# wuyakuma/HIPRT-Path-Tracer

Hardware: AMD Instinct MI355X
Metric: Mray/s + Msample/s, Bistro 1920×1080, 1/2/4/8 MI355X; RMSE vs ref @256spp (higher is better)
Workload: dtype f32

## Files before the change

hiprt-path-tracer_amd/csrc/mpt_api.cpp:

```cpp
#include <dlfcn.h>
#include <hip/hip_runtime.h>

#include <algorithm>
#include <cfloat>
#include <cmath>
#include <cstdio>
#include <cstdlib>
#include <cstring>
#include <deque>
#include <mutex>
#include <string>
#include <vector>

#include "bvh8.h"
#include "denoise.h"
#include "display.h"
#include "mpt.h"
#include "mpt_internal.h"
#include "refit.h"

using namespace mpt;

namespace {

// ... 49 lines not shown

constexpr int FRAME_RING = 256;
constexpr int PIX_PARTS_MAX = 4;
constexpr int RESTIR_MAX_BATCH = 128;
constexpr int EV_POOL = 2 * 2 * ((10 * 65 + 3 + 8) > 50 * RESTIR_MAX_BATCH ? (10 * 65 + 3 + 8) : 50 * RESTIR_MAX_BATCH);
constexpr int SPILL_WORDS = 2 * TRAV_SPILL_DEPTH;
constexpr int MAX_STACK = TRAV_LDS_STACK + TRAV_SPILL_DEPTH;

}

struct MptContext {
    int device = 0;
    hipStream_t stream = nullptr;
    bool own_stream = false;
    int overlap = -1;
    hipStream_t stream2 = nullptr;
    hipStream_t streamx[2] = {nullptr, nullptr};
    hipEvent_t ev_joinx[2] = {nullptr, nullptr};
    hipEvent_t ev_fork = nullptr, ev_first = nullptr, ev_acc = nullptr, ev_join = nullptr;
    int restir_overlap = 1;
    bool restir_overlap_ok = false;
    int restir_half = 0;
    hipEvent_t ev_chain = nullptr, ev_half[2] = {nullptr, nullptr}, ev_wave_join = nullptr;
    bool ev_half_used[2] = {false, false};
    bool wave_pending = false;
    int graphs = 0;
    int pix_parts = 3;
    int restir_side = 1;
    hipEvent_t ev_side[2] = {nullptr, nullptr};
    int trace_ahead = 1;
    int ovl_ahead = 1;
    hipEvent_t ev_ahead[2] = {nullptr, nullptr};
    hipEvent_t ev_ahead2[2] = {nullptr, nullptr};
    uint32_t ahead_launches = 0;
    uint32_t pipelined_batches = 0;
    hipGraphExec_t graph_exec = nullptr;
    std::vector<uint8_t> graph_key;
    uint32_t graph_launches = 0;
    uint32_t graph_captures = 0, graph_replays = 0;
    uint32_t overlapped_batches = 0;
    int num_cus = 256;
    int grid = 1024;
    bool has_scene = false;
    BVH8 bvh;
    DBuf<Node8> nodes;
    DBuf<TriRec> tris;
    DBuf<float4> tri_attr;
    DBuf<float> srgb;
    BVH8 bvh_light;
    DBuf<Node8> nodes_light;
    DBuf<TriRec> tris_light;
    std::vector<int32_t> h_light_prims;
    std::vector<int32_t> h_idx;
    std::vector<float> h_pos;
    float box_pad = 0.0f;
    DBuf<float> nbox, nbox_light, tbox;
    double area0 = 0.0, area0_light = 0.0;
    bool mirrors_stale = false;
    bool topology_stale = false;
    std::vector<uint8_t> h_vert_used;
    int refit_host_loop = 0;
    int light_bvh = 1;
    bool light_bvh_ok = false;
    int light_bvh_max_stack = 1 << 30;
    DBuf<int32_t> idx, mat_idx, mat_prio, emissive, tex_dims;
    DBuf<float> pos, nrm, uv;
    DBuf<uint8_t> has_n, tex;
    DBuf<uint64_t> tex_off;
    DBuf<MptMaterial> mats;
    DBuf<MptMaterial> mats_res;
    DBuf<int32_t> mat_tex;
    DBuf<float4> em_tab;
    bool any_tex = false;
    bool any_glass = false;
    double tex_tri_frac = 0.0;
    int mat_private = -1;
    int shade_classes = 1;
    int restir_staged = 1;
    int restir_mono_reuse = 0;
    int restir_batch = 1;
    int adaptive_batch = 1;
    int restir_max_batch = RESTIR_MAX_BATCH;
    int shade_glass = 1;
    int shade_split = 0;
    int shade_texmetal = 1;
    std::vector<MptMaterial> h_mats;
    std::vector<int32_t> h_mat_idx;
    std::vector<uint8_t> h_tex_alpha;
    int n_tex = 0;
    DBuf<float> lut_conductor, lut_glossy, lut_glass, lut_glass_inv, lut_thin, lut_sheen;
    DBuf<float4> env;
    DBuf<int2> alias;
    DBuf<float4> env_rich;
    DBuf<float> env_cdf;
    float env_cdf_sum = 0.0f;
    int env_w = 0, env_h = 0;
    float env_sum = 0.0f;
    int res_x = 0, res_y = 0, band_h = 1, band_i = 0, band_c = 1, n_slots = 0;
    int batch_cap = 0;
    int batch = 1;
    DBuf<float4> ray_o, ray_d, hit, thr, col, alb, nrmv, nq_o, nq_d, nhit, s_gn;
    DBuf<uint8_t> hit_inside, hit_cls, occ, qmask;
    DBuf<uint32_t> rng, spill, spill2, spillx[2];
    DBuf<uint2> seeds;
    DBuf<uint4> vsA, vsB;
    DBuf<int32_t> q0, q1, qh, qm, qf, nq_light, counters, nq_tgt, fetch_raw;
    DBuf<float4> nthr, na, nb, ndir, nris, ne1, ne2;
    DBuf<float4> nthr2, na2, nb2, ndir2, nris2, ne12, ne22, nq_o2, nq_d2, ce, ce2;
    DBuf<int32_t> nq_tgt2, qh2, qf2;
    int pipeline = 1;
    size_t pipe_n = 0;
    hipEvent_t ev_nee[4] = {nullptr, nullptr, nullptr, nullptr};
    int pix_pipe = 1;
    DBuf<float> fb_color, fb_albedo, fb_normal;
    DBuf<int32_t> as_count, as_conv;
    DBuf<float> as_sqlum;
    DBuf<uint8_t> active;
    DBuf<uint32_t> status;
    DBuf<float4> gb_pos, gb_sn, gb_gn, gb_view, pgb_pos, pgb_sn, pgb_gn, pgb_view;
    DBuf<int4> gb_meta, pgb_meta;
    DBuf<uint4> gb_vsA, gb_vsB, pgb_vsA, pgb_vsB;
    DBuf<MptMaterial> gb_mat, pgb_mat;
    DBuf<float4> gb_cs, pgb_cs;
    DBuf<float4> rs_init, rs_sp1, rs_sp2, rs_plights;
    DBuf<float4> rs_keep;
    DBuf<int32_t> rs_conv;
    DBuf<float4> rq_o, rq_d, rq_rec;
    DBuf<uint32_t> rq_key;
    DBuf<uint8_t> rq_occ;
    DBuf<int32_t> rq_list, rq_items;
    DBuf<int4> rq_meta;
    int restir_chunk = -1;
    int ci_chunk = 1;
    DBuf<float4> ci_pos, ci_sn, ci_gn, ci_view, ci_cs, ci_rs, ci_pl;
    DBuf<int4> ci_meta;
    DBuf<uint4> ci_vsA, ci_vsB;
    DBuf<MptMaterial> ci_mat;
    DevPaths ci_dp{};
    int restir_out_sp2 = 0;
    MptHaloExchangeFn halo_fn = nullptr;
    void* halo_user = nullptr;
    int halo_prev = 0;
    int32_t* h_reproj = nullptr;
    DBuf<MptMaterial> mat_slot;
    DBuf<float4> xq_o, xq_d, xq_hit, xrec;
    DBuf<uint8_t> xq_occ, xq_flag;
    DBuf<int32_t> xl_any, xl_cl, xl_light;
    int x_per = 0, x_iter = 0;
    DBuf<uint64_t> stats;
    DBuf<uint64_t> ray_counts;
    MptFrame* h_frames = nullptr;
    MptFrame* d_frames = nullptr;
    int frame_slot = 0;
    bool timing = false;
    bool instrumented = false;
    hipEvent_t ev[2][EV_POOL];
    int ev_mode[2][EV_POOL / 2];
    hipEvent_t ev_frame[2][2];
    int ev_used[2] = {0, 0};
    bool ev_pending[2] = {false, false};
    uint32_t frames_submitted = 0;
    uint32_t trace_launches = 0;
    uint32_t frames = 0;
    double stage_ms[KT_COUNT] = {};
    uint32_t stage_launches[KT_COUNT] = {};
    double frame_ms = 0.0;
// ... 619 lines not shown
    return MPT_OK;
}

int mpt_device_info(int device, char* name, int32_t name_cap, char* arch, int32_t arch_cap, int32_t* out_cus) {
    hipDeviceProp_t p;
    HIPCHK(hipGetDeviceProperties(&p, device));
    if (name && name_cap > 0) { std::strncpy(name, p.name, (size_t)name_cap - 1); name[name_cap - 1] = 0; }
    if (arch && arch_cap > 0) { std::strncpy(arch, p.gcnArchName, (size_t)arch_cap - 1); arch[arch_cap - 1] = 0; }
    if (out_cus) *out_cus = p.multiProcessorCount;
    return MPT_OK;
}

static_assert(sizeof(MptMaterial) == 332, "RendererMaterial mirror");
static_assert(sizeof(MptRenderSettings) == 304, "HIPRTRenderSettings mirror");
static_assert(sizeof(MptWorldSettings) == 200, "WorldSettings mirror");
static_assert(sizeof(MptCamera) == 196, "HIPRTCamera mirror");

int mpt_partition_rows(int32_t res_y, int32_t bh, int32_t bi, int32_t bc) {
    if (bh <= 0 || bc <= 0) return 0;
    return rows_of(res_y, bh, bi, bc);
}

static int create_context(MptContext* c, int device, void* hip_stream) {
    c->device = device;
    HIPCHK(hipSetDevice(device));
    hipDeviceProp_t prop;
    HIPCHK(hipGetDeviceProperties(&prop, device));
    c->num_cus = prop.multiProcessorCount;
    c->grid = c->num_cus * MPT_TRACE_BLOCKS_PER_CU;
    if (hip_stream) c->stream = (hipStream_t)hip_stream;
    else { HIPCHK(hipStreamCreateWithFlags(&c->stream, hipStreamNonBlocking)); c->own_stream = true; }
    HIPCHK(hipHostMalloc((void**)&c->h_frames, sizeof(MptFrame) * (FRAME_RING + 1)));
    HIPCHK(hipMalloc((void**)&c->d_frames, sizeof(MptFrame) * (FRAME_RING + 1)));
    HIPCHK(c->counters.alloc(PIX_PARTS_MAX * CTR_COUNT));
    HIPCHK(hipMemsetAsync(c->counters.p, 0, PIX_PARTS_MAX * CTR_COUNT * sizeof(int32_t), c->stream));
    HIPCHK(c->fetch_raw.alloc(4));
    HIPCHK(c->stats.alloc(N_STATS));
    HIPCHK(hipMemsetAsync(c->stats.p, 0, N_STATS * sizeof(uint64_t), c->stream));
    HIPCHK(c->ray_counts.alloc(N_RAY_COUNTS));
    HIPCHK(c->status.alloc(4));
    HIPCHK(hipMemsetAsync(c->status.p, 0, 4 * sizeof(uint32_t), c->stream));
    HIPCHK(hipMemsetAsync(c->ray_counts.p, 0, N_RAY_COUNTS * sizeof(uint64_t), c->stream));
    HIPCHK(c->spill.alloc((size_t)c->num_cus * TRACE_SPILL_BLOCKS_PER_CU * TRAV_BLOCK * SPILL_WORDS));
    HIPCHK(c->srgb.alloc(256));
    HIPCHK(launch_srgb_table(c->srgb.p, c->stream));
    return MPT_OK;
}

static int ensure_events(MptContext* c) {
    for (int p = 0; p < 2; p++) {
        for (int i = 0; i < EV_POOL; i++)
            if (!c->ev[p][i]) HIPCHK(hipEventCreate(&c->ev[p][i]));
        for (int k = 0; k < 2; k++)
            if (!c->ev_frame[p][k]) HIPCHK(hipEventCreate(&c->ev_frame[p][k]));
    }
    return MPT_OK;
}

int mpt_create(int device, void* hip_stream, MptContext** out) {
    if (!out) return fail(MPT_ERR_INVALID_ARGUMENT, "out_ctx is NULL");
    int ndev = 0;
    if (hipGetDeviceCount(&ndev) != hipSuccess || ndev <= 0) return fail(MPT_ERR_HIP, "no HIP device available");
    if (device < 0 || device >= ndev) return fail(MPT_ERR_INVALID_ARGUMENT, "device index out of range");
    MptContext* c = new MptContext();
    if (const char* e = std::getenv("MPT_SHADE_CLASSES")) c->shade_classes = std::atoi(e);
    if (const char* e = std::getenv("MPT_RESTIR_STAGED")) c->restir_staged = std::atoi(e);
    if (const char* e = std::getenv("MPT_RESTIR_MONO_REUSE")) c->restir_mono_reuse = std::atoi(e);
    if (const char* e = std::getenv("MPT_RESTIR_BATCH")) c->restir_batch = std::atoi(e);
    if (const char* e = std::getenv("MPT_ADAPTIVE_BATCH")) c->adaptive_batch = std::atoi(e);
    if (const char* e = std::getenv("MPT_MAT_PRIVATE")) c->mat_private = std::atoi(e);
    if (const char* e = std::getenv("MPT_RESTIR_OVERLAP")) c->restir_overlap = std::atoi(e);
    if (const char* e = std::getenv("MPT_GRAPHS")) c->graphs = std::atoi(e);
    if (const char* e = std::getenv("MPT_PIX_PARTS")) c->pix_parts = std::atoi(e);
    if (const char* e = std::getenv("MPT_RESTIR_SIDE")) c->restir_side = std::atoi(e);
    if (const char* e = std::getenv("MPT_TRACE_AHEAD")) c->trace_ahead = std::atoi(e);
    if (const char* e = std::getenv("MPT_PIPELINE")) c->pipeline = std::atoi(e);
    if (const char* e = std::getenv("MPT_PIX_PIPE")) c->pix_pipe = std::atoi(e);
    if (const char* e = std::getenv("MPT_OVERLAP_AHEAD")) c->ovl_ahead = std::atoi(e);
    if (const char* e = std::getenv("MPT_RESTIR_MAX_BATCH"))
        c->restir_max_batch = std::max(1, std::min(RESTIR_MAX_BATCH, std::atoi(e)));
    if (const char* e = std::getenv("MPT_RESTIR_CHUNK")) c->restir_chunk = std::atoi(e);
    if (const char* e = std::getenv("MPT_SHADE_GLASS")) c->shade_glass = std::atoi(e);
    if (const char* e = std::getenv("MPT_SHADE_SPLIT")) c->shade_split = std::atoi(e);
    if (const char* e = std::getenv("MPT_SHADE_TEXMETAL")) c->shade_texmetal = std::atoi(e);
    if (const char* e = std::getenv("MPT_LIGHT_BVH")) c->light_bvh = std::atoi(e);
    if (const char* e = std::getenv("MPT_OVERLAP")) c->overlap = std::atoi(e);
    if (const char* e = std::getenv("MPT_LIGHT_BVH_MAX_STACK")) c->light_bvh_max_stack = std::atoi(e);
    if (const char* e = std::getenv("MPT_REFIT_HOST")) c->refit_host_loop = std::atoi(e);
    int r = create_context(c, device, hip_stream);
    if (r != MPT_OK) {
        const std::string msg = g_err;
        mpt_destroy(c);
        g_err = msg;
        return r;
    }
    *out = c;
    return MPT_OK;
}

namespace {
void rccl_comm_destroy(void* comm);
}

int mpt_destroy(MptContext* c) {
    if (!c) return MPT_OK;
    (void)hipSetDevice(c->device);
    if (c->stream) (void)hipStreamSynchronize(c->stream);
    if (c->comm) rccl_comm_destroy(c->comm);
    for (int p = 0; p < 2; p++) {
        for (int i = 0; i < EV_POOL; i++)
            if (c->ev[p][i]) (void)hipEventDestroy(c->ev[p][i]);
        for (int k = 0; k < 2; k++)
            if (c->ev_frame[p][k]) (void)hipEventDestroy(c->ev_frame[p][k]);
    }
    if (c->graph_exec) (void)hipGraphExecDestroy(c->graph_exec);
    if (c->h_frames) (void)hipHostFree(c->h_frames);
    if (c->h_reproj) (void)hipHostFree(c->h_reproj);
    if (c->d_frames) (void)hipFree(c->d_frames);
    if (c->own_stream && c->stream) (void)hipStreamDestroy(c->stream);
    if (c->stream2) (void)hipStreamDestroy(c->stream2);
    for (int k = 0; k < 2; k++) {
        if (c->streamx[k]) (void)hipStreamDestroy(c->streamx[k]);
        if (c->ev_joinx[k]) (void)hipEventDestroy(c->ev_joinx[k]);
        if (c->ev_side[k]) (void)hipEventDestroy(c->ev_side[k]);
        if (c->ev_ahead[k]) (void)hipEventDestroy(c->ev_ahead[k]);
        if (c->ev_ahead2[k]) (void)hipEventDestroy(c->ev_ahead2[k]);
    }
    for (hipEvent_t e : c->ev_nee)
        if (e) (void)hipEventDestroy(e);
    for (hipEvent_t e : {c->ev_fork, c->ev_first, c->ev_acc, c->ev_join, c->ev_chain, c->ev_half[0], c->ev_half[1],
                         c->ev_wave_join})
        if (e) (void)hipEventDestroy(e);
    delete c;
    (void)hipGetLastError();
    return MPT_OK;
}

int mpt_upload_scene(MptContext* c, const MptScene* s) {
    if (!c || !s) return fail(MPT_ERR_INVALID_ARGUMENT, "NULL argument");
    if (s->num_triangles <= 0 || s->num_vertices <= 0 || !s->triangle_indices || !s->vertices || !s->material_indices ||
        !s->materials || s->num_materials <= 0)
        return fail(MPT_ERR_INVALID_ARGUMENT, "scene has no geometry or materials");
    for (int64_t i = 0; i < 3 * (int64_t)s->num_triangles; i++)
        if (s->triangle_indices[i] < 0 || s->triangle_indices[i] >= s->num_vertices)
            return fail(MPT_ERR_INVALID_ARGUMENT, "triangle index out of range");
    for (int64_t i = 0; i < s->num_triangles; i++)
        if (s->material_indices[i] < 0 || s->material_indices[i] >= s->num_materials)
            return fail(MPT_ERR_INVALID_ARGUMENT, "material index out of range");
    for (int i = 0; i < s->num_emissive_triangles; i++)
        if (s->emissive_triangle_indices[i] < 0 || s->emissive_triangle_indices[i] >= s->num_triangles)
            return fail(MPT_ERR_INVALID_ARGUMENT, "emissive triangle index out of range");
    HIPCHK(hipSetDevice(c->device));
    const int stack_cap = build_scene_bvh8(s->vertices, s->triangle_indices, s->num_triangles, c->bvh, MAX_STACK);
    c->box_pad = scene_box_pad(s->vertices, s->num_triangles, s->triangle_indices);
    c->area0 = node_box_area_sum(c->bvh.node_box.data(), c->bvh.nodes.size());
    c->mirrors_stale = false;
    c->topology_stale = false;
    c->h_vert_used.assign((size_t)s->num_vertices, 0);
    for (size_t k = 0; k < 3 * (size_t)s->num_triangles; k++) c->h_vert_used[s->triangle_indices[k]] = 1;
    c->h_idx.assign(s->triangle_indices, s->triangle_indices + 3 * (size_t)s->num_triangles);
    c->h_pos.assign(s->vertices, s->vertices + 3 * (size_t)s->num_vertices);
    c->h_light_prims.clear();
    c->nodes_light.release();
    c->tris_light.release();
    if (2 * c->bvh.depth + 2 > stack_cap) return fail(MPT_ERR_UNSUPPORTED, "BVH8 deeper than the traversal stack");
    hipStream_t st = c->stream;
// ... 437 lines not shown
        return fail(MPT_ERR_INVALID_ARGUMENT, "ReSTIR DI across a partition needs mpt_set_halo_exchange");
    if (f->options.direct_light_sampling == MPT_LSS_RESTIR_DI) {
        r = ensure_restir(c, f);
        if (r != MPT_OK) return r;
    }
    if (f->options.direct_light_sampling == MPT_LSS_RESTIR_DI && c->emissive.n == 0 &&
        (f->options.restir_di_later_bounces_sampling_strategy == MPT_RESTIR_DI_LATER_BOUNCES_UNIFORM_ONE_LIGHT ||
         f->options.restir_di_later_bounces_sampling_strategy == MPT_RESTIR_DI_LATER_BOUNCES_MIS_LIGHT_BSDF))
        return fail(MPT_ERR_UNSUPPORTED, "ReSTIR DI later bounces: uniform / MIS light sampling without emissive "
                                         "triangles picks from an empty list in the reference (Lights.h:22-220)");
    if ((int64_t)std::max(c->n_slots, 1) * batch > MPT_MAX_WAVEFRONT_PATHS)
        return fail(MPT_ERR_OUT_OF_MEMORY, "wavefront above MPT_MAX_WAVEFRONT_PATHS paths");
    const MptRenderSettings& frs = f->render_settings;
    const bool adaptive = (frs.stop_pixel_noise_threshold > 0.0f || frs.enable_adaptive_sampling) && frs.accumulate;
    const bool want_overlap = f->options.direct_light_sampling == MPT_LSS_RESTIR_DI && batch > 1 && c->restir_overlap &&
                              !(adaptive && c->as_reset_pending) &&
                              ext_layout(*f, nullptr) == 0 && (int64_t)std::max(c->n_slots, 1) * 2 * batch <= MPT_MAX_WAVEFRONT_PATHS;
    c->restir_overlap_ok = false;
    if (want_overlap) {
        const int cap = 2 * batch;
        r = ensure_batch(c, cap, c->any_tex || f->bsdf_flags.white_furnace_mode);
        if (r == MPT_OK) c->restir_overlap_ok = c->batch_cap / 2 >= batch;
        else { (void)hipGetLastError(); g_err.clear(); }
    }
    if (!c->restir_overlap_ok) {
        r = ensure_batch(c, batch, c->any_tex || f->bsdf_flags.white_furnace_mode);
        if (r != MPT_OK) return r;
    }
    const bool keep = f->options.direct_light_sampling == MPT_LSS_RESTIR_DI &&
                      f->world_settings.ambient_light_type == MPT_AMBIENT_ENVMAP;
    if (!keep && c->rs_keep.p) {
        HIPCHK(drain(c));
        c->rs_keep.release();
    }
    const size_t keep_n = 3 * (size_t)std::max(c->n_slots, 1) * (size_t)(c->restir_overlap_ok ? c->batch_cap : batch);
    if (keep && batch > 1 && c->rs_keep.n < keep_n) {
        HIPCHK(drain(c));
        c->rs_keep.release();
        if (c->rs_keep.alloc(keep_n) != hipSuccess) {
            (void)hipGetLastError();
            return fail(MPT_ERR_OUT_OF_MEMORY, "ReSTIR DI batch reservoirs");
        }
    }
    int iter = 0;
    const int per = ext_layout(*f, &iter);
    return ensure_ext(c, batch, per, iter);
}

static int ensure_overlap(MptContext* c) {
    if (c->stream2) return MPT_OK;
    if (c->spill2.n != c->spill.n) HIPCHK(c->spill2.alloc(c->spill.n));
    for (hipEvent_t* e : {&c->ev_fork, &c->ev_first, &c->ev_acc, &c->ev_join, &c->ev_chain, &c->ev_half[0], &c->ev_half[1],
                          &c->ev_wave_join})
        if (!*e) HIPCHK(hipEventCreateWithFlags(e, hipEventDisableTiming));
    HIPCHK(hipStreamCreateWithFlags(&c->stream2, hipStreamNonBlocking));
    return MPT_OK;
}

static int join_waves(MptContext* c);

static int ensure_pix_parts(MptContext* c, int parts) {
    int r = ensure_overlap(c);
    if (r != MPT_OK) return r;
    for (int k = 0; k + 2 < parts; k++) {
        if (c->spillx[k].n != c->spill.n) HIPCHK(c->spillx[k].alloc(c->spill.n));
        if (!c->ev_joinx[k]) HIPCHK(hipEventCreateWithFlags(&c->ev_joinx[k], hipEventDisableTiming));
        if (!c->streamx[k]) HIPCHK(hipStreamCreateWithFlags(&c->streamx[k], hipStreamNonBlocking));
    }
    return MPT_OK;
}

static hipError_t launch_frame_graph(MptContext* c, const DevPaths& P, const MptFrame* f, int slot, LaunchCfg& cfg) {
    const DevScene S = dev_scene(c);
    MptFrame k = *f;
    k.random_seed = 0;
    k.camera_random_seed = 0;
    std::memset(k.restir_di_seeds, 0, sizeof(k.restir_di_seeds));
    std::memset(&k.current_camera, 0, sizeof(MptCamera));
    std::memset(&k.prev_camera, 0, sizeof(MptCamera));
    k.render_settings.sample_number = 0;
    k.render_settings.denoiser_AOV_accumulation_counter = 0;
    k.render_settings.need_to_reset = false;
    k.render_settings.do_update_status_buffers = false;
    const int flags[9] = {cfg.grid_persistent, cfg.stats, cfg.shade_classes, cfg.light_bvh, cfg.light_static,
                          cfg.restir_staged, cfg.shade_glass, cfg.shade_split, cfg.mat_private};
    std::vector<uint8_t> key(sizeof(k) + sizeof(S) + sizeof(P) + sizeof(flags));
    uint8_t* q = key.data();
    std::memcpy(q, &k, sizeof(k)); q += sizeof(k);
    std::memcpy(q, &S, sizeof(S)); q += sizeof(S);
    std::memcpy(q, &P, sizeof(P)); q += sizeof(P);
    std::memcpy(q, flags, sizeof(flags));
    MptFrame* d_fixed = c->d_frames + FRAME_RING;
    hipError_t e = hipMemcpyAsync(d_fixed, c->h_frames + slot, sizeof(MptFrame), hipMemcpyHostToDevice, c->stream);
    if (e != hipSuccess) return e;
    if (!c->graph_exec || key != c->graph_key) {
        if (c->graph_exec) { (void)hipGraphExecDestroy(c->graph_exec); c->graph_exec = nullptr; }
        hipGraph_t g = nullptr;
        e = hipStreamBeginCapture(c->stream, hipStreamCaptureModeThreadLocal);
        if (e != hipSuccess) return e;
        LaunchCfg gc = cfg;
        gc.launches = 0;
        const hipError_t le = launch_frame(S, P, d_fixed, *f, gc, c->stream);
        e = hipStreamEndCapture(c->stream, &g);
        if (le != hipSuccess || e != hipSuccess) {
            if (g) (void)hipGraphDestroy(g);
            (void)hipGetLastError();
            c->graphs = 0;
            return launch_frame(S, P, c->d_frames + slot, *f, cfg, c->stream);
        }
        e = hipGraphInstantiate(&c->graph_exec, g, nullptr, nullptr, 0);
        (void)hipGraphDestroy(g);
        if (e != hipSuccess) {
            c->graph_exec = nullptr;
            (void)hipGetLastError();
            c->graphs = 0;
            return launch_frame(S, P, c->d_frames + slot, *f, cfg, c->stream);
        }
        c->graph_key = std::move(key);
        c->graph_launches = gc.launches;
        c->graph_captures++;
    }
    cfg.launches += c->graph_launches;
    c->graph_replays++;
    return hipGraphLaunch(c->graph_exec, c->stream);
}

static bool is_reset(const MptFrame& f) { return f.render_settings.sample_number == 0 || f.render_settings.need_to_reset; }
static bool has_adaptive(const MptFrame& f) {
    const MptRenderSettings& rs = f.render_settings;
    return (rs.stop_pixel_noise_threshold > 0.0f || rs.enable_adaptive_sampling) && rs.accumulate;
}
static int next_as_bound(int b, const MptFrame& f) {
    if (!has_adaptive(f)) return b;
    if (is_reset(f)) b = 0;
    return b < (1 << 30) ? b + 1 : b;
}
static bool note_conv_set(bool set, int bound, const MptFrame& f) {
    if (!has_adaptive(f)) return set;
    const MptRenderSettings& rs = f.render_settings;
    if (is_reset(f)) { set = false; bound = 0; }
    if (rs.enable_adaptive_sampling) return set || bound > rs.adaptive_sampling_min_samples;
    return set || (rs.enable_pixel_stop_noise_threshold && rs.sample_number > 1);
}
static int set_ahead(MptContext* c, LaunchCfg& cfg, const MptFrame& f, int which = 0) {
    if (!c->trace_ahead || f.render_settings.nb_bounces <= 0) return MPT_OK;
    int rr = ensure_pix_parts(c, 4);
    if (rr != MPT_OK) return rr;
    hipEvent_t* evs = which ? c->ev_ahead2 : c->ev_ahead;
    for (int k = 0; k < 2; k++)
        if (!evs[k]) HIPCHK(hipEventCreateWithFlags(&evs[k], hipEventDisableTiming));
    cfg.ahead_stream = which ? c->streamx[0] : c->streamx[1];
    cfg.ahead_spill = which ? c->spillx[0].p : c->spillx[1].p;
    cfg.ev_ahead_fork = evs[0];
    cfg.ev_ahead_join = evs[1];
    return MPT_OK;
}

static bool pipe_applies(const MptContext* c, const MptFrame& f) {
    return c->pipeline && f.options.direct_light_sampling != MPT_LSS_RESTIR_DI && c->x_per == 0 && !c->shade_split &&
           f.render_settings.nb_bounces > 0;
}
static int set_pipe(MptContext* c, LaunchCfg& cfg, const MptFrame& f, DevPaths& P, DevPaths& alt, int part = -1,
                    size_t off = 0) {
    if (!pipe_applies(c, f)) return MPT_OK;
    const size_t N = (size_t)std::max(c->n_slots, 1) * (size_t)c->batch_cap;
    if (c->pipe_n != N) {
        HIPCHK(drain(c));
        Allocs A;
// ... 18 lines not shown
    alt = P;
    alt.nthr = c->nthr2.p; alt.na = c->na2.p; alt.nb = c->nb2.p; alt.ndir = c->ndir2.p; alt.nris = c->nris2.p;
    alt.ne1 = c->ne12.p; alt.ne2 = c->ne22.p; alt.nq_o = c->nq_o2.p; alt.nq_d = c->nq_d2.p; alt.nq_tgt = c->nq_tgt2.p;
    alt.qh = c->qh2.p; alt.qf = c->qf2.p; alt.ce = c->ce2.p;
    if (off) {
        alt.nthr += off; alt.na += off; alt.nb += off; alt.ndir += off; alt.nris += off; alt.ne1 += off; alt.ne2 += off;
        alt.nq_o += off; alt.nq_d += off; alt.nq_tgt += 4 * off; alt.qh += off; alt.qf += off; alt.ce += off;
    }
    alt.counters = part < 0 ? P.counters + CTR_COUNT : P.counters + 2 * CTR_COUNT;
    cfg.pipe_alt = &alt;
    cfg.nee_stream = c->streamx[k];
    cfg.nee_spill = c->spillx[k].p;
    cfg.ev_nee_fork = c->ev_nee[2 * k];
    cfg.ev_nee_join = c->ev_nee[2 * k + 1];
    return MPT_OK;
}

static int launch_batch(MptContext* c, const MptFrame* f, int batch) {
    const bool restir_part = f->options.direct_light_sampling == MPT_LSS_RESTIR_DI && f->band_count > 1;
    if (!(f->options.direct_light_sampling == MPT_LSS_RESTIR_DI && batch > 1 && c->restir_overlap_ok)) {
        int jr = join_waves(c);
        if (jr != MPT_OK) return jr;
    }
    const int parts_set = c->pix_pipe && pipe_applies(c, *f) ? std::min(c->pix_parts, 2) : c->pix_parts;
    const int parts = std::min(std::max(parts_set, 1), std::min(PIX_PARTS_MAX, f->res_y));
    const bool pix_ovl = parts > 1 && batch == 1 && f->band_count == 1 && c->n_slots >= (1 << 16) &&
                         f->options.direct_light_sampling != MPT_LSS_RESTIR_DI && c->x_per == 0 &&
                         !(c->graphs && !c->timing);
    const int nfr = batch + (pix_ovl ? parts - 1 : 0);
    if (c->frame_slot + nfr > FRAME_RING) c->frame_slot = 0;
    int slot = c->frame_slot;
    c->frame_slot = (c->frame_slot + nfr) % FRAME_RING;
    if (slot == 0) {
        HIPCHK(hipStreamSynchronize(c->stream));
        if (c->stream2) HIPCHK(hipStreamSynchronize(c->stream2));
    }
    for (int k = 0; k < batch; k++) c->h_frames[slot + k] = f[k];
    const int hp = (f->res_y + parts - 1) / parts;
    if (pix_ovl) {
        for (int k = 1; k < parts; k++) {
            MptFrame& g = c->h_frames[slot + k];
            g = f[0];
            g.band_height = hp;
            g.band_index = k;
            g.band_count = parts;
        }
    }
    HIPCHK(hipMemcpyAsync(c->d_frames + slot, c->h_frames + slot, nfr * sizeof(MptFrame), hipMemcpyHostToDevice,
                          c->stream));
    int pool = (int)(c->frames_submitted & 1u);
    if (c->timing) {
        int rc = collect_pool(c, pool);
        if (rc != MPT_OK) return rc;
    }
    LaunchCfg cfg{};
    cfg.grid_persistent = c->grid;
    cfg.stats = c->instrumented ? 1 : 0;
    cfg.ev_pool = c->timing ? c->ev[pool] : nullptr;
    cfg.ev_mode = c->ev_mode[pool];
    cfg.ev_cap = EV_POOL;
    cfg.ev_used = 0;
    cfg.restir_out_sp2 = c->restir_out_sp2;
    cfg.shade_classes = c->shade_classes;
    cfg.restir_staged = c->restir_staged;
    cfg.restir_mono_reuse = c->restir_mono_reuse;
    if (c->ci_chunk > 1 && c->ci_pos.p && c->ci_pl.n >= 4 * (size_t)std::max(1, f->render_settings.restir_di_settings.number_of_subsets *
                                                                                     f->render_settings.restir_di_settings.subset_size) * c->ci_chunk) {
        cfg.ci_chunk = c->ci_chunk;
        cfg.ci_planes = &c->ci_dp;
    }
    if (f->options.direct_light_sampling == MPT_LSS_RESTIR_DI && c->restir_staged &&
        (c->restir_side > 1 || (c->restir_side == 1 && c->n_slots <= (1 << 20)))) {
        int rr = ensure_pix_parts(c, 3);
        if (rr != MPT_OK) return rr;
        for (hipEvent_t& ev : c->ev_side)
            if (!ev) HIPCHK(hipEventCreateWithFlags(&ev, hipEventDisableTiming));
        cfg.side_stream = c->streamx[0];
        cfg.side_spill = c->spillx[0].p;
        cfg.ev_side_fork = c->ev_side[0];
        cfg.ev_side_join = c->ev_side[1];
    }
    cfg.shade_glass = c->shade_glass && c->any_glass;
    cfg.shade_split = c->shade_split;
    cfg.mat_private = c->mat_private >= 0 ? (c->mat_private != 0) : (c->tex_tri_frac >= 0.25);
    cfg.light_bvh = c->light_bvh && c->light_bvh_ok;
    cfg.light_static = !c->h_light_prims.empty() && 2 * c->bvh_light.depth + 2 <= TRAV_LDS_STACK;
    if (restir_part) {
        if (!c->h_reproj) HIPCHK(hipHostMalloc((void**)&c->h_reproj, sizeof(int32_t), hipHostMallocDefault));
        cfg.halo_fn = c->halo_fn;
        cfg.halo_user = c->halo_user;
        cfg.own_y0 = f->band_index * f->band_height;
        cfg.own_y1 = std::min(f->res_y, cfg.own_y0 + f->band_height);
        cfg.halo_prev = c->halo_prev;
        cfg.halo_rows = c->halo_prev;
        cfg.h_reproj = c->h_reproj;
    }
    if (c->timing) HIPCHK(hipEventRecord(c->ev_frame[pool][0], c->stream));
    c->batch = batch;
    DevPaths P = dev_paths(c);
    c->batch = 1;
    {
        const MptRenderSettings& rs = f->render_settings;
        P.spec_as = batch > 1 && (rs.stop_pixel_noise_threshold > 0.0f || rs.enable_adaptive_sampling) && rs.accumulate;
        P.spec_skip = P.spec_as && rs.enable_adaptive_sampling && c->as_bound > rs.adaptive_sampling_min_samples;
    }
    if (restir_part) {
        P.rs_lo = std::max(0, cfg.own_y0 - cfg.halo_prev) * f->res_x;
        P.rs_hi = std::min(f->res_y, cfg.own_y1 + cfg.halo_prev) * f->res_x;
    }
    const bool pipe_ok = c->pipeline && !c->shade_split && f->render_settings.nb_bounces > 0;
    const bool pipe_first = pipe_ok && c->mat_idx.n >= PIPELINE_PREFER_TRIS;
    const bool ovl_auto = ((size_t)batch * (size_t)std::max(c->n_slots, 1) <= OVERLAP_AUTO_PATHS && !pipe_first) ||
                          (f->render_settings.nb_bounces >= 8 && !pipe_ok);
    const bool ovl = (c->overlap > 0 || (c->overlap < 0 && ovl_auto)) && batch >= 2 &&
                     f->options.direct_light_sampling != MPT_LSS_RESTIR_DI && c->x_per == 0 && !P.spec_as;
    hipError_t e = hipSuccess;
    if (pix_ovl) {
        int rr = ensure_pix_parts(c, parts);
        if (rr != MPT_OK) return rr;
        HIPCHK(hipEventRecord(c->ev_fork, c->stream));
        LaunchCfg cur = cfg;
        int launches = 0;
        const bool part_pipe = c->pix_pipe && parts == 2 && pipe_applies(c, *f);
        DevPaths alts[2];
        for (int k = 0; k < parts && e == hipSuccess; k++) {
            const size_t r0 = std::min((size_t)f->res_y, (size_t)k * hp), r1 = std::min((size_t)f->res_y, (size_t)(k + 1) * hp);
            const size_t off = r0 * (size_t)f->res_x, n = (r1 - r0) * (size_t)f->res_x;
            if (n == 0) continue;
            DevPaths Pk = P;
            Pk.n = Pk.n_pix = (int)n;
            if (k > 0) {
                offset_slots(Pk, off);
                Pk.fb_color += 3 * off; Pk.fb_albedo += 3 * off; Pk.fb_normal += 3 * off;
                Pk.as_count += off; Pk.as_sqlum += off; Pk.as_conv += off;
                Pk.counters += k * CTR_COUNT;
                Pk.stack_spill = k == 1 ? c->spill2.p : c->spillx[k - 2].p;
            }
            hipStream_t sk = k == 0 ? c->stream : k == 1 ? c->stream2 : c->streamx[k - 2];
            if (k > 0) HIPCHK(hipStreamWaitEvent(sk, c->ev_fork, 0));
            cur.pipe_alt = nullptr;
            cur.nee_stream = nullptr;
            if (part_pipe) {
                int rr2 = set_pipe(c, cur, *f, Pk, alts[k], k, k > 0 ? off : 0);
                if (rr2 != MPT_OK) return rr2;
                if (cur.pipe_alt) c->pipelined_batches++;
            }
            cur.launches = 0;
            e = launch_frame(dev_scene(c), Pk, c->d_frames + slot + k, k == 0 ? f[0] : c->h_frames[slot + k], cur, sk);
            launches += cur.launches;
        }
        for (int k = 1; k < parts; k++) {
            hipStream_t sk = k == 1 ? c->stream2 : c->streamx[k - 2];
            hipEvent_t ej = k == 1 ? c->ev_join : c->ev_joinx[k - 2];
            HIPCHK(hipEventRecord(ej, sk));
            HIPCHK(hipStreamWaitEvent(c->stream, ej, 0));
        }
        c->overlapped_batches++;
        cfg.ev_used = cur.ev_used;
        cfg.launches = launches;
    } else if (ovl) {
        int rr = ensure_overlap(c);
        if (rr != MPT_OK) return rr;
        const int b0 = batch / 2, b1 = batch - b0;
        c->batch = b0;
        DevPaths P0 = dev_paths(c);
        c->batch = b1;
// ... 559 lines not shown
        const int p0 = std::min(res_y, p * bh), p1 = std::min(res_y, p0 + bh);
        int c0, c1, d0, d1, lo, hi;
        const bool theirs = need(p, c0, c1, d0, d1);
        for (int i = 0; i < n_buffers; i++) {
            if (theirs && band_overlap(c0, c1, m0, m1, lo, hi)) ops.push_back({p, 0, i, lo, hi});
            if (theirs && band_overlap(d0, d1, m0, m1, lo, hi)) ops.push_back({p, 0, i, lo, hi});
            if (mine && band_overlap(a0, a1, p0, p1, lo, hi)) ops.push_back({p, 1, i, lo, hi});
            if (mine && band_overlap(b0, b1, p0, p1, lo, hi)) ops.push_back({p, 1, i, lo, hi});
        }
    }
}
int native_halo(void* user, MptHaloExchange* x) {
    MptContext* c = (MptContext*)user;
    hipStream_t st = (hipStream_t)x->stream;
    std::vector<MptHaloOp>& ops = c->halo_plan_ops;
    auto count = [&](int recv) {
        size_t bytes = 0;
        for (const MptHaloOp& o : ops)
            if (o.recv == recv) bytes += (size_t)(o.row_hi - o.row_lo) * (size_t)x->res_x * (size_t)x->bytes_per_pixel[o.buffer];
        return bytes;
    };
    if (c->halo_native == 2) {
        if (x->phase == MPT_HALO_GBUFFER && !x->halo_agreed && hipStreamSynchronize(st) != hipSuccess) return 1;
        halo_ops(x->res_y, c->band_h, std::max(1, c->band_c), c->band_i, x->halo_rows, x->n_buffers, ops);
        const size_t bytes = count(1);
        c->halo_exchanges++;
        c->halo_bytes_recv += bytes;
        c->halo_bytes_sent += count(0);
        if (bytes == 0) return 0;
        if (c->halo_scratch.n < 2 * bytes && c->halo_scratch.alloc(2 * bytes) != hipSuccess) return 1;
        return hipMemcpyAsync(c->halo_scratch.p + bytes, c->halo_scratch.p, bytes, hipMemcpyDeviceToDevice, st) == hipSuccess ? 0 : 1;
    }
    Rccl& r = *rccl_lib();
    if (!c->comm || !r.send || !r.recv || !r.group_start || !r.group_end || !r.all_reduce) return 2;
    const int n = c->comm_size, k = c->comm_rank;
    if (c->band_c != n || c->band_i != k) return 4;
    if (x->phase == MPT_HALO_GBUFFER && !x->halo_agreed) {
        if (c->halo_agree.n < 1 && c->halo_agree.alloc(1) != hipSuccess) return 1;
        int32_t v = x->halo_rows;
        if (hipMemcpyAsync(c->halo_agree.p, &v, sizeof(v), hipMemcpyHostToDevice, st) != hipSuccess) return 1;
        if (r.all_reduce(c->halo_agree.p, c->halo_agree.p, 1, NCCL_INT32, NCCL_MAX, c->comm, st) != 0) return 3;
        if (hipMemcpyAsync(&v, c->halo_agree.p, sizeof(v), hipMemcpyDeviceToHost, st) != hipSuccess ||
            hipStreamSynchronize(st) != hipSuccess) return 1;
        x->halo_rows = v;
        c->halo_agreements++;
    }
    halo_ops(x->res_y, c->band_h, n, k, x->halo_rows, x->n_buffers, ops);
    c->halo_exchanges++;
    c->halo_bytes_recv += count(1);
    c->halo_bytes_sent += count(0);
    if (ops.empty()) return 0;
    int rc = r.group_start();
    for (size_t j = 0; j < ops.size() && rc == 0; j++) {
        const MptHaloOp& o = ops[j];
        uint8_t* buf = (uint8_t*)x->buffers[o.buffer];
        const size_t row = (size_t)x->res_x * (size_t)x->bytes_per_pixel[o.buffer];
        uint8_t* at = buf + (size_t)o.row_lo * row;
        const size_t len = (size_t)(o.row_hi - o.row_lo) * row;
        rc = o.recv ? r.recv(at, len, NCCL_UINT8, o.peer, c->comm, st) : r.send(at, len, NCCL_UINT8, o.peer, c->comm, st);
    }
    const int re = r.group_end();
    return rc != 0 ? 3 : (re != 0 ? 3 : 0);
}
}

int mpt_halo_plan(int32_t res_y, int32_t band_height, int32_t band_count, int32_t band_index, int32_t halo_rows,
                  int32_t n_buffers, MptHaloOp* out, int32_t cap) {
    if (res_y <= 0 || band_height <= 0 || band_count <= 0 || band_index < 0 || band_index >= band_count || halo_rows < 0 ||
        n_buffers < 0 || n_buffers > MPT_HALO_MAX_BUFFERS || cap < 0 || (cap > 0 && !out))
        return fail(MPT_ERR_INVALID_ARGUMENT, "mpt_halo_plan: bad partition, halo or output");
    std::vector<MptHaloOp> ops;
    halo_ops(res_y, band_height, band_count, band_index, halo_rows, n_buffers, ops);
    for (size_t j = 0; j < ops.size() && (int32_t)j < cap; j++) out[j] = ops[j];
    return (int)ops.size();
}

int mpt_set_pipeline(MptContext* c, int32_t mode) {
    if (!c) return fail(MPT_ERR_INVALID_ARGUMENT, "NULL context");
    if (mode < 0 || mode > 1) return fail(MPT_ERR_INVALID_ARGUMENT, "mode must be 0 (in line) or 1 (pipelined)");
    c->pipeline = mode;
    return MPT_OK;
}

int mpt_set_halo_native(MptContext* c, int32_t mode) {
    if (!c) return fail(MPT_ERR_INVALID_ARGUMENT, "NULL context");
    if (mode < 0 || mode > 2) return fail(MPT_ERR_INVALID_ARGUMENT, "mode must be 0 (off), 1 (RCCL) or 2 (rehearsal)");
    if (mode == 1) {
        if (!c->comm) return fail(MPT_ERR_INVALID_ARGUMENT, "no communicator (mpt_comm_init)");
        Rccl& r = *rccl_lib();
        if (!r.send || !r.recv || !r.group_start || !r.group_end || !r.all_reduce)
            return fail(MPT_ERR_UNSUPPORTED, "librccl.so.1 lacks ncclSend / ncclRecv / ncclGroupStart / ncclAllReduce");
    }
    c->halo_native = mode;
    c->halo_fn = mode ? &native_halo : nullptr;
    c->halo_user = mode ? (void*)c : nullptr;
    return MPT_OK;
}

int mpt_clear_status(MptContext* c) {
    if (!c) return fail(MPT_ERR_INVALID_ARGUMENT, "NULL context");
    HIPCHK(hipSetDevice(c->device));
    HIPCHK(hipMemsetAsync(c->status.p, 0, 4 * sizeof(uint32_t), c->stream));
    return MPT_OK;
}

int mpt_query_status(MptContext* c, MptStatus* out) {
    if (!c || !out) return fail(MPT_ERR_INVALID_ARGUMENT, "NULL argument");
    HIPCHK(hipSetDevice(c->device));
    uint32_t v[4];
    HIPCHK(hipMemcpyAsync(v, c->status.p, sizeof(v), hipMemcpyDeviceToHost, c->stream));
    HIPCHK(hipStreamSynchronize(c->stream));
    out->one_ray_active = v[1] != 0;
    out->pixel_converged_count = v[0];
    return MPT_OK;
}

int mpt_get_aux_buffer(MptContext* c, int kind, void* dst, int dst_is_device) {
    if (!c || !dst) return fail(MPT_ERR_INVALID_ARGUMENT, "NULL argument");
    const void* src = kind == MPT_AUX_SAMPLE_COUNT ? (const void*)c->as_count.p
                    : kind == MPT_AUX_CONVERGED_SAMPLE_COUNT ? (const void*)c->as_conv.p
                    : kind == MPT_AUX_SQUARED_LUMINANCE ? (const void*)c->as_sqlum.p : nullptr;
    size_t bytes = (size_t)c->n_slots * 4;
    if (kind >= MPT_AUX_RESTIR_OUTPUT && kind <= MPT_AUX_RESTIR_INITIAL && c->rs_init.p) {
        const int o = c->restir_out_sp2;
        const float4* out = o == 1 ? c->rs_sp2.p : o == 2 ? c->rs_init.p : c->rs_sp1.p;
        src = kind == MPT_AUX_RESTIR_OUTPUT ? (const void*)out
            : kind == MPT_AUX_RESTIR_OTHER ? (const void*)(o == 1 ? c->rs_sp1.p : c->rs_sp2.p) : (const void*)c->rs_init.p;
        bytes = c->rs_init.n * sizeof(float4);
    }
    if (!src) return fail(MPT_ERR_INVALID_ARGUMENT, "bad aux buffer kind or no frame rendered");
    HIPCHK(hipSetDevice(c->device));
    HIPCHK(hipMemcpyAsync(dst, src, bytes, dst_is_device ? hipMemcpyDeviceToDevice : hipMemcpyDeviceToHost, c->stream));
    HIPCHK(hipStreamSynchronize(c->stream));
    return MPT_OK;
}

int mpt_enable_stats(MptContext* c, int enable, int instrumented) {
    if (!c) return fail(MPT_ERR_INVALID_ARGUMENT, "NULL context");
    HIPCHK(hipSetDevice(c->device));
    HIPCHK(hipStreamSynchronize(c->stream));
    if (enable) {
        int r = ensure_events(c);
        if (r != MPT_OK) { c->timing = false; return r; }
    }
    c->timing = enable != 0;
    c->instrumented = instrumented != 0;
    c->ev_pending[0] = c->ev_pending[1] = false;
    c->trace_launches = 0;
    c->frames = 0;
    c->frame_ms = 0.0;
    c->graph_captures = c->graph_replays = 0;
    c->overlapped_batches = 0;
    c->halo_exchanges = c->halo_agreements = c->halo_bytes_sent = c->halo_bytes_recv = 0;
    c->restir_overlapped_batches = 0;
    c->ahead_launches = 0;
    c->pipelined_batches = 0;
    for (int m = 0; m < KT_COUNT; m++) { c->stage_ms[m] = 0.0; c->stage_launches[m] = 0; }
    HIPCHK(hipMemsetAsync(c->stats.p, 0, N_STATS * sizeof(uint64_t), c->stream));
    HIPCHK(hipMemsetAsync(c->ray_counts.p, 0, N_RAY_COUNTS * sizeof(uint64_t), c->stream));
    HIPCHK(hipStreamSynchronize(c->stream));
    return MPT_OK;
}

int mpt_get_stats(MptContext* c, MptStats* out) {
    if (!c || !out) return fail(MPT_ERR_INVALID_ARGUMENT, "NULL argument");
    HIPCHK(hipSetDevice(c->device));
// ... 157 lines not shown
```

hiprt-path-tracer_amd/csrc/mpt_internal.h:

```cpp
#ifndef MPT_INTERNAL_H
#define MPT_INTERNAL_H

#include <hip/hip_runtime.h>
#include <stdint.h>

#include "bvh8.h"
#include "mpt.h"

namespace mpt {

constexpr int TRAV_BLOCK = 256;
#ifndef MPT_LDS_STACK
#define MPT_LDS_STACK 12
#endif
constexpr int TRAV_LDS_STACK = MPT_LDS_STACK;
constexpr int TRAV_SPILL_DEPTH = 64 - TRAV_LDS_STACK;

#ifndef MPT_TRACE_BLOCKS_PER_CU
#define MPT_TRACE_BLOCKS_PER_CU 5
#endif
#ifndef MPT_TRACE_WAVES
#define MPT_TRACE_WAVES 5
#endif
#ifndef MPT_TRACE_WAVES_LIST
// ... 102 lines not shown
    float4* nq_d;
    int64_t nq_stride;
    int32_t* nq_tgt;
    uint8_t* qmask;
    uint8_t* occ;
    float4* nhit;
    float4* s_gn;
    MptMaterial* mat_slot;
    float4* ce;
    float* fb_color;
    float* fb_albedo;
    float* fb_normal;
    uint32_t* stack_spill;
    uint64_t* stats;
    uint64_t* ray_counts;
    int32_t* as_count;
    float* as_sqlum;
    int32_t* as_conv;
    uint8_t* active;
    int32_t spec_as;
    int32_t spec_reset;
    int32_t spec_skip;
    uint32_t* status;
    float4* gb_pos;
    float4* gb_sn;
    float4* gb_gn;
    float4* gb_view;
    int4* gb_meta;
    uint4* gb_vsA;
    uint4* gb_vsB;
    MptMaterial* gb_mat;
    float4* pgb_pos; float4* pgb_sn; float4* pgb_gn; float4* pgb_view; int4* pgb_meta;
    uint4* pgb_vsA; uint4* pgb_vsB; MptMaterial* pgb_mat;
    float4* gb_cs; float4* pgb_cs;
    float4* rs_init;
    float4* rs_sp1;
    float4* rs_sp2;
    float4* rs_out;
    float4* rs_tin;
    float4* rs_keep;
    int64_t rs_keep_n;
    int rs_keep_on;
    int32_t cam_noqueue;
    float4* rs_plights;
    int32_t pix_off;
    int32_t rs_lo, rs_hi;
    int32_t ci_n;
    int32_t ci_pix_off;
    int32_t* rs_conv;
    int32_t x_per;
    int32_t x_iter;
    float4* xq_o;
    float4* xq_d;
    float4* xq_hit;
    uint8_t* xq_occ;
    uint8_t* xq_flag;
    float4* xrec;
    int32_t* xl_any;
    int32_t* xl_cl;
    int32_t* xl_light;
    float4* rq_o;
    float4* rq_d;
    uint32_t* rq_key;
    uint8_t* rq_occ;
    int32_t* rq_list;
    int32_t* rq_items;
    int4* rq_meta;
    float4* rq_rec;
};

constexpr int N_TRACE_MODES = 5;
constexpr int RS_KMAX_HOST = 5, RS_RPP_HOST = 2 * RS_KMAX_HOST + 2, RS_REC_HOST = RS_KMAX_HOST + 2;
constexpr int N_RAY_COUNTS = 6;
enum { KT_CAMERA = 3, KT_SHADE = 4, KT_RESOLVE = 5, KT_ACCUMULATE = 6, KT_COMPACT = 7, KT_RESTIR = 8, KT_SPLIT = 9,
       KT_MISS = 10, KT_SHADE_GENERIC = 11,
       KT_GBUFFER = 12, KT_RS_PRESAMPLE = 13, KT_RS_INITIAL = 14, KT_RS_REUSE = 15, KT_RS_SPATIAL = 16,
       KT_RS_EVAL = 17, KT_COUNT = 18 };
constexpr uint32_t QM_CONT = 16u;
constexpr int32_t MT_TEXTURED = 1, MT_FULL = 2, MT_GLASS = 4;
constexpr int32_t MT_TEXMETAL = 8;
constexpr int STATS_STRIDE = 6;
constexpr int N_STATS = N_TRACE_MODES * STATS_STRIDE;

enum {
    CTR_Q0 = 0, CTR_Q1 = 1,
    CTR_QG = 2,
    CTR_ANY = 3, CTR_CL = 4,
    CTR_FETCH = 5,
    CTR_REPROJ = 6,
    CTR_HIT = 7, CTR_MISS = 8,
    CTR_FULL = 9,
    CTR_DEFER = 10,
    CTR_LIGHT = 11,
    CTR_XANY = 12, CTR_XCL = 13, CTR_XLIGHT = 14,
    CTR_RQ = 15, CTR_RQV = 16,
    CTR_RQE0 = 17, CTR_RQE1 = 18,
    CTR_F_RQA = 19, CTR_F_RQB = 20,
    CTR_RQ_GROUP = 6,
    CTR_GLASS = 21,
    CTR_F_PATH = 22, CTR_F_ANY = 23, CTR_F_CL = 24, CTR_F_OCC = 25, CTR_F_XANY = 26, CTR_F_XCL = 27, CTR_F_XOCC = 28,
    CTR_COUNT = 29
};
constexpr int CTR_BOUNCE_FIRST = CTR_ANY;

struct LaunchCfg {
    int grid_persistent;
    int stats;
    hipEvent_t* ev_pool;
    int* ev_mode;
    int ev_cap;
    int ev_used;
    uint32_t launches;
    int restir_out_sp2;
    MptHaloExchangeFn halo_fn;
    void* halo_user;
    int own_y0, own_y1;
    int halo_prev;
    int halo_rows;
    int32_t* h_reproj;
    int halo_rc;
    int shade_classes;
    int light_bvh;
    int light_static;
    int restir_staged;
    int restir_mono_reuse;
    int shade_glass;
    int mat_private;
    int shade_split;
    hipEvent_t ev_first_trace;
    hipEvent_t ev_acc_done;
    hipEvent_t ev_acc_wait;
    hipStream_t wave_stream;
    uint32_t* wave_spill;
    hipEvent_t ev_chain;
    hipStream_t side_stream;
    uint32_t* side_spill;
    hipEvent_t ev_side_fork, ev_side_join;
    hipStream_t ahead_stream;
    uint32_t* ahead_spill;
    hipEvent_t ev_ahead_fork, ev_ahead_join;
    uint32_t ahead_launches;
    hipStream_t nee_stream;
    uint32_t* nee_spill;
    hipEvent_t ev_nee_fork, ev_nee_join;
    const DevPaths* pipe_alt;
    int ci_chunk;
    const DevPaths* ci_planes;
};

inline void offset_slots(DevPaths& P, size_t off) {
    P.ray_o += off; P.ray_d += off; P.hit += off; P.hit_inside += off; P.hit_cls += off; P.rng += off; P.seeds += off; P.thr += off; P.col += off;
    P.vsA += off; P.vsB += off; P.alb += off; P.nrm += off;
    P.q0 += off; P.q1 += off; P.qh += off; P.qm += off; P.qf += off; P.nq_light += off;
    P.nthr += off; P.na += off; P.nb += off; P.ndir += off; P.nris += off; P.ne1 += off; P.ne2 += off;
    P.nq_o += off; P.nq_d += off; P.occ += off; P.nq_tgt += 4 * off;
    P.nhit += off; P.s_gn += off; P.qmask += off; P.active += off;
    if (P.mat_slot) P.mat_slot += off;
    if (P.ce) P.ce += off;
}

hipError_t launch_frame(const DevScene& S, const DevPaths& P, const MptFrame* d_frame, const MptFrame& h_frame,
                        LaunchCfg& cfg, hipStream_t st);
hipError_t launch_frames_restir(const DevScene& S, const DevPaths& P, const MptFrame* d_frames, const MptFrame* h_frames,
                                int batch, LaunchCfg& cfg, hipStream_t st);
hipError_t launch_resolve_materials(const DevScene& S, MptMaterial* out_res, int32_t* out_tex, int n, float4* em_tab,
                                   hipStream_t st);
hipError_t launch_restir_fill(float4* reservoirs, int n, hipStream_t st);
hipError_t launch_restir_fill_lights(float4* lights, int n, hipStream_t st);
hipError_t launch_bake(int kind, int w, int h, int d, int ipk, int nb_samples, int iteration, float* out, hipStream_t st);
hipError_t launch_tri_attr(const DevScene& S, float4* out, hipStream_t st);
hipError_t launch_srgb_table(float* out, hipStream_t st);
hipError_t launch_env_rich(const DevScene& S, float4* out, hipStream_t st);
hipError_t launch_display(const MptDisplaySettings& S, const float* src, const float* src2, const int32_t* cnt, int W,
                          int rows, uint32_t* dst, hipStream_t st);
size_t denoise_scratch_floats(int64_t pixels);
hipError_t launch_denoise(const MptDenoiseSettings& S, const float* color, const float* albedo, const float* normals,
                          int W, int H, float* scratch, float* dst, hipStream_t st);
hipError_t launch_refit_tris(TriRec* tris, int n, const int32_t* idx, const float* pos, float pad, float* tbox, hipStream_t st);
hipError_t launch_refit_levels(Node8* nodes, float* node_box, const float* tbox, const int32_t* level_begin, int levels,
                               hipStream_t st);
int build_scene_bvh8(const float* vertices, const int32_t* indices, int32_t num_triangles, BVH8& out, int stack_limit);
int copy_bvh_out(const Node8* nodes, size_t n_nodes, const TriRec* tris, size_t n_tris, int levels, void* out_nodes,
                 int64_t nodes_cap, void* out_tris, int64_t tris_cap, int32_t* out_counts);
struct LbvhDevice {
    Node8* nodes = nullptr;
    TriRec* tris = nullptr;
    float* nbox = nullptr;
    int n_nodes = 0, n_tris = 0, depth = 0;
    std::vector<int32_t> level_begin;
};
struct PlocStats {
    int iterations = 0, tail_iterations = 0;
};
hipError_t build_lbvh_device(const int32_t* d_prims, int n, int n_scene_prims, const int32_t* idx, const float* pos, float pad,
                             const TriRec* old_tris, int n_old, float* tbox, LbvhDevice& out, hipStream_t st, int mode = 0,
                             PlocStats* stats = nullptr);
void free_lbvh(LbvhDevice& o);
hipError_t scan_u64(uint64_t* a, int n, uint64_t* partial, hipStream_t st);
struct PlocScratch {
    int32_t* cref[2];
    int32_t* ccnt[2];
    float* cbox[2];
    int32_t* mate;
    uint64_t* words;
    uint64_t* partial;
    int32_t* count;
    int32_t* tail_info;
};
hipError_t ploc_tree_device(int n, const float* pbox, const uint32_t* order, int32_t* left, int32_t* right, int32_t* first,
                            int32_t* last, float* nbox, uint32_t* order_out, const PlocScratch& B, hipStream_t st,
// ... 33 lines not shown
```

hiprt-path-tracer_amd/csrc/mpt_kernels.hip:

```cpp
#include <hip/hip_runtime.h>

#include <cfloat>
#include <cstring>
#include <initializer_list>
#include <type_traits>
#include <utility>

#include "dev_bsdf.h"
#include "mpt_internal.h"

namespace mpt {

constexpr int TB = TRAV_BLOCK;
constexpr int MAX_BOUNDARY_SKIPS = 16;
#ifndef MPT_TRACE_REFILL
#define MPT_TRACE_REFILL 32
#endif
#ifndef MPT_TRACE_BUDGET
#define MPT_TRACE_BUDGET 16
#endif
constexpr int TRACE_REFILL = MPT_TRACE_REFILL;
constexpr int TRACE_BUDGET = MPT_TRACE_BUDGET;
#ifndef MPT_TRACE_CHUNK
#define MPT_TRACE_CHUNK 256
// ... 1134 lines not shown
                    x_rec(P, ew, make_float4(fw_.r, fw_.g, fw_.b, maxr(0.0f, dot(sn, Lw))), make_float4(0.0f, 0.0f, 0.0f, 0.0f));
                    fw |= XQ_REC;
                    if (vis && ism != 1.0f) x_query(P, ew, true, ep2, prim, Lw, dw - 1.0e-4f, fw);
                }
                if (!vis) {
                    const float cw = inner ? w * target / lpdf : 0.0f;
                    wsum += cw;
                    if (r < cw / wsum) { win = c; win_L = Lw; win_d = dw; }
                }
                P.xq_flag[e] = f0;
                P.xq_flag[ew] = fw;
            }
            if (!vis && win >= 0) {
                uint8_t fw = XQ_REC;
                x_query(P, e0 + nl + win, true, ep2, prim, win_L, win_d - 1.0e-4f, fw);
                P.xq_flag[e0 + nl + win] = fw;
            }
            for (int b = 0; b < nbc; b++) {
                uint8_t fb = 0;
                const size_t e = e0 + 2 * nl + b;
                const float pdf = x_bsdf_cand<OVR, FULL>(P, bc, m, vs, pe, e, prim, ip, sn, gn, view, ism, ep, true, 0.0f, rng, fb);
                const float r = rng();
                if (pdf > 0.0f) P.xrec[2 * e + 1].y = r;
                else x_rec(P, e, make_float4(0.0f, 0.0f, 0.0f, 0.0f), make_float4(0.0f, r, 0.0f, 0.0f));
                P.xq_flag[e] = fb | XQ_REC;
            }
        }
    }
}

DEV void store3(float* p, Col c) { p[0] = c.r; p[1] = c.g; p[2] = c.b; }
DEV void store3(float* p, v3 c) { p[0] = c.x; p[1] = c.y; p[2] = c.z; }
DEV Col load3c(const float* p) { return col(p[0], p[1], p[2]); }
DEV v3 load3v(const float* p) { return mk3(p[0], p[1], p[2]); }

#ifdef MPT_SECTION_TIMING
static __device__ unsigned long long g_sect[8];
#define SECT_BEGIN() uint64_t sect_[6] = {0, 0, 0, 0, 0, 0}; uint64_t tprev_ = __builtin_amdgcn_s_memtime()
#define SECT(k) do { uint64_t now_ = __builtin_amdgcn_s_memtime(); sect_[k] += now_ - tprev_; tprev_ = now_; } while (0)
#define SECT_END() do { if (sect_[1]) for (int k_ = 0; k_ < 6; k_++) atomicAdd(&g_sect[k_], (unsigned long long)sect_[k_]); atomicAdd(&g_sect[7], 1ull); } while (0)
#else
#define SECT_BEGIN() do {} while (0)
#define SECT(k) do {} while (0)
#define SECT_END() do {} while (0)
#endif

enum : uint32_t { RF_ENVMAP = 1u, RF_BSDF_REFRACTION = 2u, RF_UNOCCLUDED = 4u };
struct RResv { int M; float wsum; float UCW; int tri; v3 point; float target; uint32_t flags; };
DEV RResv rr_default() {
    RResv r;
    r.M = 0; r.wsum = 0.0f; r.UCW = 0.0f; r.tri = -1; r.point = mk3(0.0f, 0.0f, 0.0f); r.target = 0.0f; r.flags = 0u;
    return r;
}
DEV RResv rr_load(const float4* b, int i) {
    float4 a = b[3 * (size_t)i], c = b[3 * (size_t)i + 1], d = b[3 * (size_t)i + 2];
    RResv r;
    r.M = __float_as_int(a.x); r.wsum = a.y; r.UCW = a.z; r.tri = __float_as_int(a.w);
    r.point = mk3(c.x, c.y, c.z); r.target = c.w; r.flags = __float_as_uint(d.x);
    return r;
}
DEV void rr_store(float4* b, int i, const RResv& r) {
    b[3 * (size_t)i] = make_float4(__int_as_float(r.M), r.wsum, r.UCW, __int_as_float(r.tri));
    b[3 * (size_t)i + 1] = make_float4(r.point.x, r.point.y, r.point.z, r.target);
    b[3 * (size_t)i + 2] = make_float4(__uint_as_float(r.flags), 0.0f, 0.0f, 0.0f);
}

DEV Col miss_radiance(const DevScene& S, const MptFrame& F, int bounce, v3 d, Col thr) {
    const MptRenderSettings& rs = F.render_settings;
    const MptWorldSettings& ws = F.world_settings;
    Col sky = col(0.0f);
    if (ws.ambient_light_type == MPT_AMBIENT_UNIFORM || F.bsdf_flags.white_furnace_mode) sky = C3(ws.uniform_light_color);
    else if (ws.ambient_light_type == MPT_AMBIENT_ENVMAP) {
        bool sampled = F.options.envmap_sampling != MPT_ESS_NO_SAMPLING;
        if (!sampled || bounce == 0) {
            sky = eval_env_no_pdf(S, F, d);
            bool unscale = sampled ? !ws.envmap_scale_background_intensity : (!ws.envmap_scale_background_intensity && bounce == 0);
            if (unscale) sky /= ws.envmap_intensity;
        }
    }
    sky = clamp_contrib(sky, rs.envmap_contribution_clamp, true);
    return clamp_contrib(sky * thr, rs.indirect_contribution_clamp, bounce > 0);
}

enum ShadeOp {
    OP_DONE = 0, OP_RIS_LIGHT, OP_RIS_BSDF, OP_RIS_WIN, OP_MIS_LIGHT, OP_MIS_BSDF, OP_UNI_LIGHT, OP_BSDF_LIGHT,
    OP_ENV_LIGHT, OP_ENV_BSDF, OP_CONT, OP_RESTIR
};
enum { SG_LIGHT = 1, SG_ENV = 2, SG_CONT = 4, SG_ALL = 7 };
DEV constexpr int op_group(int op) {
    return op == OP_DONE ? 0 : (op == OP_ENV_LIGHT || op == OP_ENV_BSDF) ? SG_ENV : op == OP_CONT ? SG_CONT : SG_LIGHT;
}
template <int ST>
DEV int stage_op(int op, bool do_env, bool do_cont) {
    if (!(ST & SG_LIGHT) && op_group(op) == SG_LIGHT) op = do_env ? OP_ENV_LIGHT : (do_cont ? OP_CONT : OP_DONE);
    if (!(ST & SG_ENV) && op_group(op) == SG_ENV) op = do_cont ? OP_CONT : OP_DONE;
    if (!(ST & SG_CONT) && op == OP_CONT) op = OP_DONE;
    return op;
}

struct ShadeArgs {
    DevScene S;
    DevPaths P;
    const MptFrame* F;
    int bounce;
    int last_bounce;
    int32_t* q_cur;
    const int32_t* count_cur;
    int32_t* q_defer;
    int32_t* count_defer;
    int force_defer;
    int rev;
    int mat_private;
};

#ifndef MPT_PLAIN_SAMPLE_PE
#define MPT_PLAIN_SAMPLE_PE 1
#endif
#ifndef MPT_SHADE_WAVES
#define MPT_SHADE_WAVES 2
#endif
#ifndef MPT_SHADE_PEP
#define MPT_SHADE_PEP 0
#endif
#ifndef MPT_SHADE_WAVES_PLAIN
#define MPT_SHADE_WAVES_PLAIN MPT_SHADE_WAVES
#endif
#define OPIS(X) ((ST & op_group(X)) && op == (X))
#ifndef MPT_SHADE_WAVES_LATE
#define MPT_SHADE_WAVES_LATE 3
#endif
#ifndef MPT_SHADE_PE_LDS_LATE
#define MPT_SHADE_PE_LDS_LATE 0
#endif
template <int OVR, bool PLAIN, bool EXT = false, bool GLASS = false, int ST = SG_ALL, bool MATP = false>
__global__ __launch_bounds__(TB) __attribute__((amdgpu_waves_per_eu(
    !(ST & SG_LIGHT) ? MPT_SHADE_WAVES_LATE : (PLAIN ? MPT_SHADE_WAVES_PLAIN : MPT_SHADE_WAVES)))) void k_shade(ShadeArgs A) {
    constexpr int CLS = PLAIN ? BC_PLAIN : (GLASS ? BC_GLASS : BC_FULL);
    constexpr bool PE_PLAIN = MPT_SHADE_PEP && PLAIN && OVR == MPT_BSDF_NONE && !EXT;
    constexpr bool FIRST = (ST & SG_LIGHT) != 0;
    constexpr bool LAST = (ST & SG_CONT) != 0;
    static_assert(!EXT || ST == SG_ALL, "extended light sampling shades in one stage");
    const DevScene& S = A.S;
    const DevPaths& P = A.P;
    const MptFrame& F = *A.F;
    const MptRenderSettings& rs = F.render_settings;
    const int bounce = A.bounce;
    const int count = *A.count_cur;
    if ((int)(blockIdx.x * TB) >= count) return;
    int i = blockIdx.x * TB + threadIdx.x;
    bool valid = i < count;
    int slot = valid ? (A.rev ? A.q_cur[-1 - i] : A.q_cur[i]) : 0;
    if (!FIRST && slot < 0) { valid = false; slot = 0; }

    BCtx bc;
    bc.mats = S.mats;
    bc.luts = DevLuts{S.lut_conductor, S.lut_glossy, S.lut_glass, S.lut_glass_inv, S.lut_thin_glass, S.lut_sheen};
    bc.clearcoat_comp = F.bsdf_flags.clearcoat_compensation_approximation;
    bc.masking = F.bsdf_flags.ggx_masking_shadowing;

    bool cont = false;
    SECT_BEGIN();
    if (valid) {
        float4 ro = ld_s(&P.ray_o[slot]), rdv = ld_s(&P.ray_d[slot]), hv = ld_s(&P.hit[slot]);
        v3 o = mk3(ro.x, ro.y, ro.z), d = mk3(rdv.x, rdv.y, rdv.z);
        int prim = (int)__float_as_uint(hv.w);
        bool found = prim >= 0;
        VState vs = vs_load_s(P.vsA, P.vsB, slot);
        Rng rng = make_rng(ld_s(&P.rng[slot]));
        const float4 thv = ld_s(&P.thr[slot]);
        Col thr = col(thv.x, thv.y, thv.z);
        const Col thr_vertex = thr;
        Col rcol = col(0.0f);
        if (!P.ce) {
            const float4 cv = ld_s(&P.col[slot]);
            rcol = col(cv.x, cv.y, cv.z);
        }
        v3 ip = mk3(0, 0, 0), gn = mk3(0, 0, 0), sn = mk3(0, 0, 0);
        const Mat* mp = S.mats_res;
        bool mat_in_slot = false;
        constexpr bool MAT_PRIV = MATP && ST == SG_ALL;
        Mat mat_priv;
        if (!FIRST) {
            const float4 ra = ld_s(&P.nhit[slot]), rb = ld_s(&P.s_gn[slot]);
            sn = mk3(ra.x, ra.y, ra.z);
            gn = mk3(rb.x, rb.y, rb.z);
            const int mref = __float_as_int(ra.w);
            mp = mref < 0 ? &P.mat_slot[slot] : &S.mats_res[mref];
            ip = o + hv.x * d;
            if (bounce == 0) d = normalize(d);
        } else if (found) {
            float t = hv.x;
            v2 uv = mk2(hv.y, hv.z);
            ip = o + t * d;
            const HitAttr ha = hit_attributes(S, prim, uv);
            const v2 tc = ha.tc;
            gn = ha.gn;
            sn = ha.sn;
            const int mi = ha.mi;
            if (F.bsdf_flags.white_furnace_mode || (S.mat_tex[mi] & MT_TEXTURED)) {
                if (MAT_PRIV) {
                    mat_priv = intersection_material(S, mi, tc, F.bsdf_flags.white_furnace_mode);
                    mp = &mat_priv;
                } else {
                    P.mat_slot[slot] = intersection_material(S, mi, tc, F.bsdf_flags.white_furnace_mode);
                    mp = &P.mat_slot[slot];
                }
                mat_in_slot = true;
            } else {
                mp = &S.mats_res[mi];
            }
            const Mat& m = *mp;
            bool was_inside = P.hit_inside[slot] != 0;
            if ((!was_inside || m.specular_transmission == 0.0f) && !m.thin_walled) {
                gn *= dot(gn, -d) < 0.0f ? -1.0f : 1.0f;
                sn *= dot(sn, gn) < 0.0f ? -1.0f : 1.0f;
                float NoV = dot(sn, -d);
                sn += (2.0f * clampr(0.0f, 1.0f, -NoV)) * -d;
            }
            if (m.dispersion_scale > 0.0f && m.specular_transmission > 0.0f && vs.wl == 0.0f)
                vs.wl = -(rng() * (float)(830 - 360) + (float)360);
        }
        const Mat& m = *mp;
        if (FIRST && bounce == 0) {
            if (found && is_emissive(m) && dot(-d, gn) < 0) { gn = -gn; sn = -sn; }
            gn = normalize(gn);
            sn = normalize(sn);
            d = normalize(d);
            rng = make_rng(P.seeds[slot].y);
        }
        if (PLAIN && FIRST) {
            const v3 sn_f = (is_emissive(m) && dot(-d, gn) < 0) ? -sn : sn;
            if (!(dot(-d, sn_f) > 0 || m.thin_walled) || m.metallic != 0.0f || A.force_defer || (PE_PLAIN && !plain_vertex_ok(m))) {
                A.q_defer[atomicAdd(A.count_defer, 1)] = slot;
                atomicAdd(&P.counters[CTR_DEFER], 1);
                A.q_cur[i] = -1;
                return;
            }
        }
        uint32_t fl = 0;
        uint32_t qm = 0;
        if (found) {
            if (FIRST && bounce == 0) {
                float4 a = P.alb[slot], n4 = P.nrm[slot];
                P.alb[slot] = make_float4(a.x + m.base_color.r, a.y + m.base_color.g, a.z + m.base_color.b, 0.0f);
                P.nrm[slot] = make_float4(n4.x + sn.x, n4.y + sn.y, n4.z + sn.z, 0.0f);
            }
            if (FIRST && is_emissive(m) && dot(-d, gn) < 0) { gn = -gn; sn = -sn; }
            v3 view = -d;
            if (FIRST) fl |= NF_SHADED;
            const int lss = F.options.direct_light_sampling;
            const MptWorldSettings& ws = F.world_settings;
            const bool restir = lss == MPT_LSS_RESTIR_DI;
            bool do_light = (S.n_emissive != 0 || (restir && ws.ambient_light_type == MPT_AMBIENT_ENVMAP)) &&
                            !(F.bsdf_flags.white_furnace_mode && F.bsdf_flags.white_furnace_mode_turn_off_emissives);
            if (do_light && is_emissive(m)) {
                do_light = false;
                if (FIRST && m.emissive_texture_used && bounce > 0) {
                    fl |= NF_IMM;
                    const Col e = emission_of(m);
                    st_s(&P.na[slot], make_float4(e.r, e.g, e.b, 0.0f));
                }
            }
            do_light = do_light && lss != MPT_LSS_NO_DIRECT_LIGHT_SAMPLING;
            const int lssb = bounce_lss(F, bounce);
            if (restir && bounce > 0 && S.n_emissive == 0 && lssb == MPT_LSS_RIS_BSDF_AND_LIGHT) do_light = false;
            if (FIRST && do_light) fl |= NF_L;
            const bool do_env = ws.ambient_light_type == MPT_AMBIENT_ENVMAP && !F.bsdf_flags.white_furnace_mode &&
                                !is_emissive(m) && ws.envmap_intensity > 0.0f && F.options.envmap_sampling != MPT_ESS_NO_SAMPLING &&
                                !(restir && bounce == 0);
            const bool env_use = lss != MPT_LSS_NO_DIRECT_LIGHT_SAMPLING;
            const bool do_cont = bounce < A.last_bounce;
            const float ism = dot(view, gn) < 0 ? -1.0f : 1.0f;
            const v3 ep = ip + sn * 1.0e-4f * ism;
            const int nl = rs.ris_number_of_light_candidates, nbc = rs.ris_number_of_bsdf_candidates;
            int op = OP_DONE;
            if (do_light) {
                if (restir && bounce == 0) op = OP_RESTIR;
                else if (lssb == MPT_LSS_RIS_BSDF_AND_LIGHT) op = nl > 0 ? OP_RIS_LIGHT : (nbc > 0 ? OP_RIS_BSDF : OP_RIS_WIN);
                else if (lssb == MPT_LSS_MIS_LIGHT_BSDF) op = OP_MIS_LIGHT;
                else if (lssb == MPT_LSS_UNIFORM_ONE_LIGHT) op = OP_UNI_LIGHT;
                else if (lssb == MPT_LSS_BSDF) op = OP_BSDF_LIGHT;
            }
            if (op == OP_DONE) op = do_env ? OP_ENV_LIGHT : (do_cont ? OP_CONT : OP_DONE);
            op = stage_op<ST>(op, do_env, do_cont);
            float wsum = 0.0f, targetW = 0.0f;
            v3 pointW = mk3(0, 0, 0);
            int triW = -1, ris_c = 0;
            bool hasW = false;
            float r_add = 0.0f;
            constexpr bool PE_LDS = (ST & SG_LIGHT) || MPT_SHADE_PE_LDS_LATE;
            using PE = typename std::conditional<PE_PLAIN, PEvalP, PEval>::type;
            __shared__ PE pe_lds[PE_LDS ? TB : 1];
            PE pe_reg;
            PE& pe = PE_LDS ? pe_lds[threadIdx.x] : pe_reg;
            EmPrefetch pf;
            pf.valid = false;
            if (MPT_EM_PREFETCH && (ST & SG_LIGHT) && (op == OP_RIS_LIGHT || op == OP_MIS_LIGHT || op == OP_UNI_LIGHT)) pf.issue(S, rng);
            SECT(0);
            bsdf_eval_pre<OVR, CLS>(bc, m, vs, view, sn, pe);
            SECT(5);
            if constexpr (EXT) {
                if (do_light && !(restir && bounce == 0)) {
                    ext_light<OVR, CLS>(S, P, F, bc, m, vs, pe, slot, prim, ip, sn, gn, view, ism, ep, lssb, rng);
                    fl |= NF_EXT;
                    op = do_env ? OP_ENV_LIGHT : (do_cont ? OP_CONT : OP_DONE);
                }
            }
            Col fW = col(0.0f);
            float pdfW = 0.0f;
            while (op != OP_DONE) {
                VState tv = vs;
                RResv rres;
                v3 L = mk3(0.0f, 0.0f, 0.0f);
                bool do_eval = false;
                float lpdf = 0.0f, dist = 0.0f, geo = 0.0f;
                LightInfo li;
                li.tri = -1; li.emission = col(0.0f);
                v3 lp = mk3(0.0f, 0.0f, 0.0f);
                Col ec = col(0.0f);
                bool inner = false;
                float4 etex = make_float4(0.0f, 0.0f, 0.0f, 0.0f);
                if (OPIS(OP_RIS_BSDF) || OPIS(OP_MIS_BSDF) || OPIS(OP_BSDF_LIGHT) || OPIS(OP_ENV_BSDF) || OPIS(OP_CONT)) {
                    do_eval = (MPT_PLAIN_SAMPLE_PE && CLS == BC_PLAIN && OVR == MPT_BSDF_NONE)
                                  ? principled_sample_dir_plain(bc, m, tv, pe, view, sn, gn, L, rng)
                                  : bsdf_sample_dir<OVR, CLS>(bc, m, tv, view, sn, gn, L, rng);
                    if (MPT_ENV_EARLY && OPIS(OP_ENV_BSDF) && do_eval) etex = env_fetch(S, F, L);
                } else if (OPIS(OP_RIS_LIGHT)) {
                    lp = pf.sample(S, rng, lpdf, li);
                    if (MPT_EM_PREFETCH && ris_c + 1 < nl) {
                        Rng nx = rng;
                        (void)nx();
                        pf.issue(S, nx);
                    }
                    if (lpdf > 0.0f) {
                        v3 tl = lp - ep;
                        dist = length(tl);
                        tl = tl / dist;
                        float cl = absr(dot(li.normal, -tl));
                        geo = maxr(0.0f, dot(sn * ism, tl));
                        if (geo > 0.0f && cl > 1.0e-6f) {
                            inner = true;
                            lpdf *= dist * dist;
                            lpdf /= cl;
                            if (min_contrib(rs.minimum_light_contribution, li.emission / lpdf)) { L = tl; do_eval = true; }
                        }
                    }
                } else if (OPIS(OP_RIS_WIN)) {
                    v3 ep2 = ip + sn * 1.0e-4f;
                    v3 sd = pointW - ep2;
                    dist = length(sd);
                    L = sd / dist;
                    lp = ep2;
                    do_eval = hasW && ism != 1.0f;
                } else if (OPIS(OP_MIS_LIGHT) || OPIS(OP_UNI_LIGHT)) {
                    lp = pf.sample(S, rng, lpdf, li);
                    if (lpdf > 0.0f) {
                        v3 so = OPIS(OP_MIS_LIGHT) ? ep : ip + sn * 1.0e-4f;
                        v3 sd = lp - so;
                        dist = length(sd);
                        L = sd / dist;
                        geo = absr(dot(li.normal, -L));
                        lp = so;
                        do_eval = geo > 0.0f;
                    }
                } else if (OPIS(OP_RESTIR)) {
                    float4* rsb = P.rs_out;
                    size_t rpix = (size_t)slot + P.pix_off;
                    if (P.rs_keep_on) {
                        int kpix, ksub;
                        batch_split(P, slot, kpix, ksub);
                        rsb = P.rs_keep + (size_t)ksub * 3 * (size_t)P.rs_keep_n;
                        rpix = (size_t)kpix;
                    }
                    rres = rr_load(rsb, (int)rpix);
                    if ((rres.flags & RF_ENVMAP) && ws.ambient_light_type != MPT_AMBIENT_ENVMAP) {
                        rres.UCW = 0.0f;
                        float4 a = rsb[3 * rpix];
                        rsb[3 * rpix] = make_float4(a.x, a.y, 0.0f, a.w);
                    }
                    if (rres.UCW > 0.0f) {
                        if (rres.flags & RF_ENVMAP) { L = mat_x_vec(ws.envmap_to_world_matrix.m, rres.point); dist = 1.0e35f; }
                        else { L = rres.point - ip; dist = length(L); L = L / dist; }
                        do_eval = true;
                    }
                } else if (OPIS(OP_ENV_LIGHT)) {
// ... 86 lines not shown
                        stage_query(P, slot, 3, qm, no, prim, L, 1.0e35f - 1.0e-4f);
                        st_s(&P.nb[slot], make_float4(f.r, f.g, f.b, pdf));
                        st_s(&P.ndir[slot], make_float4(L.x, L.y, L.z, maxr(0.0f, dot(sn, L))));
                    }
                } else if (OPIS(OP_RESTIR)) {
                    if (do_eval) {
                        float c = dot(sn, L);
                        if (rres.flags & RF_BSDF_REFRACTION) c = absr(c);
                        if (c > 0.0f) {
                            Col e;
                            if (rres.flags & RF_ENVMAP) { float ep_; e = env_eval(S, F, L, ep_); }
                            else e = emission_of(S.mats[S.mat_idx[rres.tri]]);
                            const Col a = f * rres.UCW * e * c;
                            st_s(&P.na[slot], make_float4(a.r, a.g, a.b, 0.0f));
                            fl |= NF_A;
                            if (!(rres.flags & RF_UNOCCLUDED) && rs.restir_di_settings.do_final_shading_visibility) {
                                fl |= NF_AQ;
                                stage_query(P, slot, 0, qm, ip, prim, L, dist - 1.0e-4f);
                            }
                        }
                    }
                } else if (OPIS(OP_ENV_LIGHT)) {
                    if (do_eval) {
                        float mw = F.options.envmap_bsdf_mis ? balance(lpdf, pdf) : 1.0f;
                        const Col e1 = f * geo * mw * ec / lpdf;
                        st_s(&P.ne1[slot], make_float4(e1.r, e1.g, e1.b, 0.0f));
#ifdef MPT_DEBUG_SLOT
                        if (slot == MPT_DEBUG_SLOT) { Col e1_ = f * geo * mw * ec / lpdf; printf("GPU env f %a %a %a bp %a mw %a e1 %a %a %a\n", f.r, f.g, f.b, pdf, mw, e1_.r, e1_.g, e1_.b); }
#endif
                        if (env_use) {
                            fl |= NF_E1;
                            stage_query(P, slot, 1, qm, ip, prim, L, 1.0e35f - 1.0e-4f);
                        }
                    }
                    next = F.options.envmap_bsdf_mis ? OP_ENV_BSDF : OP_DONE;
                } else if (OPIS(OP_ENV_BSDF)) {
                    float c2 = absr(dot(sn, L));
                    if (pdf > 0.0f) {
                        float epdf;
                        Col er = MPT_ENV_EARLY ? env_eval_tex(S, F, L, etex, epdf) : env_eval(S, F, L, epdf);
                        if (epdf > 0.0f && env_use) {
                            float mw = balance(pdf, epdf);
                            const Col e2 = er * mw * c2 * f / pdf;
                            st_s(&P.ne2[slot], make_float4(e2.r, e2.g, e2.b, 0.0f));
                            fl |= NF_E2;
                            stage_query(P, slot, 2, qm, ip, prim, L, 1.0e35f - 1.0e-4f);
                        }
                    }
                } else if (OPIS(OP_CONT)) {
#ifdef MPT_DEBUG_SLOT
                    if (slot == MPT_DEBUG_SLOT) printf("GPU b%d cont mi %d vs %d %d %d %d st %x %x %x L %a %a %a f %a %a %a pdf %a\n", bounce, (int)(mp - S.mats_res), tv.incident, tv.outgoing, (int)tv.inside, tv.pos, tv.st[0], tv.st[1], tv.st[2], L.x, L.y, L.z, f.r, f.g, f.b, pdf);
#endif
                    vs = tv;
                    Col att = f * absr(dot(L, sn)) / pdf;
                    if (!(pdf <= 0.0f)) {
                        bool alive = true;
                        if (bounce >= rs.russian_roulette_min_depth && rs.use_russian_roulette) {
                            float sp;
                            if (rs.path_russian_roulette_method == 0) sp = maxc(thr);
                            else sp = sqrtf(maxc(thr * att) / maxc(thr));
                            sp = minr(sp, 1.0f);
                            if (rng() > sp) alive = false;
                            else {
                                float inc = 1.0f / sp;
                                if (rs.russian_roulette_throughput_clamp > 0.0f) inc = minr(inc, rs.russian_roulette_throughput_clamp);
                                thr *= inc;
                            }
                        }
                        if (alive) {
                            thr *= dispersion_ray_color(vs.wl, m.dispersion_scale);
                            thr *= att;
                            st_s(&P.ray_o[slot], make_float4(ip.x, ip.y, ip.z, __uint_as_float((uint32_t)prim)));
                            st_s(&P.ray_d[slot], make_float4(L.x, L.y, L.z, INFINITY));
                            cont = true;
                        }
                    }
                    next = -1;
                }
                if (next == OP_DONE && op != OP_ENV_LIGHT && op != OP_ENV_BSDF && do_env) next = OP_ENV_LIGHT;
                else if (next == OP_DONE && do_cont) next = OP_CONT;
                op = next < 0 ? OP_DONE : stage_op<ST>(next, do_env, do_cont);
                SECT(3);
            }
            if (FIRST && lss == MPT_LSS_NO_DIRECT_LIGHT_SAMPLING) {
                Col he = clamp_contrib(emission_of(m), rs.indirect_contribution_clamp, bounce > 0);
                rcol += he * thr_vertex;
                fl &= ~(NF_A | NF_B | NF_E1 | NF_E2 | NF_RIS_W | NF_IMM | NF_L);
                fl |= NF_NOADD;
            } else if (FIRST && bounce == 0) {
                rcol += emission_of(m);
            }
            if (FIRST && !LAST) {
                const int mref = mat_in_slot ? -1 : (int)(mp - S.mats_res);
                st_s(&P.nhit[slot], make_float4(sn.x, sn.y, sn.z, __int_as_float(mref)));
                st_s(&P.s_gn[slot], make_float4(gn.x, gn.y, gn.z, 0.0f));
            }
        } else {
            rcol += miss_radiance(S, F, bounce, d, thr);
        }
        const uint32_t qb = qm | (cont ? QM_CONT : 0u);
        if (FIRST) {
            st_s(&P.nthr[slot], make_float4(thr_vertex.r, thr_vertex.g, thr_vertex.b, __uint_as_float(fl)));
            st_s(&P.qmask[slot], (uint8_t)qb);
            st_s(P.ce ? &P.ce[slot] : &P.col[slot], make_float4(rcol.r, rcol.g, rcol.b, 0.0f));
        } else {
            if (fl) {
                const float4 t4 = ld_s(&P.nthr[slot]);
                st_s(&P.nthr[slot], make_float4(t4.x, t4.y, t4.z, __uint_as_float(__float_as_uint(t4.w) | fl)));
            }
            if (qb) st_s(&P.qmask[slot], (uint8_t)(ld_s(&P.qmask[slot]) | qb));
        }
        st_s(&P.rng[slot], rng.s);
        if (LAST) st_s(&P.thr[slot], make_float4(thr.r, thr.g, thr.b, 0.0f));
        if (FIRST || LAST) vs_store_s(P.vsA, P.vsB, slot, vs);
    }
    SECT(4);
    SECT_END();
}

#ifndef MPT_TU_PART
__global__ __launch_bounds__(TB) void k_miss(DevScene S, DevPaths P, const MptFrame* __restrict__ Fp, int bounce) {
    const int nm = P.counters[CTR_MISS];
    for (int i = blockIdx.x * TB + threadIdx.x; i < nm; i += gridDim.x * TB) {
        const int slot = P.qm[i];
        const float4 rdv = ld_s(&P.ray_d[slot]), t4 = ld_s(&P.thr[slot]), cv = ld_s(&P.col[slot]);
        v3 d = mk3(rdv.x, rdv.y, rdv.z);
        if (bounce == 0) d = normalize(d);
        const Col rc = col(cv.x, cv.y, cv.z) + miss_radiance(S, *Fp, bounce, d, col(t4.x, t4.y, t4.z));
        st_s(&P.col[slot], make_float4(rc.r, rc.g, rc.b, 0.0f));
    }
}

#endif
constexpr int CP_NT = 1024;
constexpr int CP_ITEMS = 8;

DEV int block_scan_excl(int v, int* tmp, int& total) {
    const int lane = lane_id(), wid = threadIdx.x >> 6;
    constexpr int NW = CP_NT / 64;
    int x = v;
#pragma unroll
    for (int o = 1; o < 64; o <<= 1) {
        int y = __shfl_up(x, o);
        if (lane >= o) x += y;
    }
    if (lane == 63) tmp[wid] = x;
    __syncthreads();
    if (wid == 0) {
        int w = lane < NW ? tmp[lane] : 0;
        int xs = w;
#pragma unroll
        for (int o = 1; o < NW; o <<= 1) {
            int y = __shfl_up(xs, o);
            if (lane >= o) xs += y;
        }
        if (lane < NW) tmp[lane] = xs - w;
        if (lane == NW - 1) tmp[NW] = xs;
    }
    __syncthreads();
    int excl = x - v + tmp[wid];
    total = tmp[NW];
    __syncthreads();
    return excl;
}

DEV int load_items(const int32_t* q, int b0, int count, int slots[CP_ITEMS]) {
    const int i0 = b0 + (int)threadIdx.x * CP_ITEMS;
    const int n = max(0, min(CP_ITEMS, count - i0));
    if (n == CP_ITEMS) {
        const int4 a = *reinterpret_cast<const int4*>(q + i0), b = *reinterpret_cast<const int4*>(q + i0 + 4);
        slots[0] = a.x; slots[1] = a.y; slots[2] = a.z; slots[3] = a.w;
        slots[4] = b.x; slots[5] = b.y; slots[6] = b.z; slots[7] = b.w;
    } else {
#pragma unroll
        for (int j = 0; j < CP_ITEMS; j++) slots[j] = j < n ? q[i0 + j] : 0;
    }
    return n;
}

#ifndef MPT_TU_PART
__global__ __launch_bounds__(CP_NT) void k_split(DevScene S, DevPaths P, const int32_t* q, const int32_t* count_q,
                                                 int classes, int32_t* zero_next) {
    __shared__ int tmp[CP_NT / 64 + 1];
    __shared__ int base[4];
    const int count = *count_q;
// ... 365 lines not shown
    if (invalid) {
        if (rs.display_NaNs) {
            Col dc = col(1.0e30f, 0.0f, 1.0e30f);
            if (rs.sample_number != 0) dc = dc * (float)rs.sample_number;
            f.c = dc;
        }
        return;
    }
    any = true;
    if (has_adaptive_buffers(rs)) {
        float l = lum(c);
        f.sq += l * l;
    }
    if (rs.sample_number == 0) f.c = c;
    else { f.c.r += c.r; f.c.g += c.g; f.c.b += c.b; }
    float cnt = (float)rs.denoiser_AOV_accumulation_counter;
    float4 a = P.alb[slot], n = P.nrm[slot];
    if (rs.sample_number == 0) {
        f.a = mk3(a.x, a.y, a.z);
        f.n = mk3(n.x, n.y, n.z);
    } else {
        f.a.x = (f.a.x * cnt + a.x) / (cnt + 1.0f);
        f.a.y = (f.a.y * cnt + a.y) / (cnt + 1.0f);
        f.a.z = (f.a.z * cnt + a.z) / (cnt + 1.0f);
        v3 acc = (f.n * cnt + mk3(n.x, n.y, n.z)) / (cnt + 1.0f);
        float len = length(acc);
        if (!is_zero(len)) f.n = acc / len;
    }
}
#ifndef MPT_TU_PART
__global__ __launch_bounds__(TB) void k_accumulate(DevPaths P, const MptFrame* __restrict__ Fp) {
    const int pixel = blockIdx.x * TB + threadIdx.x;
    bool any = false;
    uint32_t n_conv = 0u;
    if (pixel < P.n_pix) {
        float* fb = P.fb_color + 3 * (size_t)pixel;
        float* fa = P.fb_albedo + 3 * (size_t)pixel;
        float* fn = P.fb_normal + 3 * (size_t)pixel;
        PixAcc f;
        f.c = col(fb[0], fb[1], fb[2]);
        f.a = mk3(fa[0], fa[1], fa[2]);
        f.n = mk3(fn[0], fn[1], fn[2]);
        bool adaptive = false;
        for (int sub = 0; sub < P.batch; sub++) adaptive |= has_adaptive_buffers(Fp[sub].render_settings);
        f.sq = adaptive ? P.as_sqlum[pixel] : 0.0f;
        if (P.spec_as) {
            int cnt = P.as_count[pixel], conv = P.as_conv[pixel];
            for (int sub = 0; sub < P.batch; sub++) {
                const MptRenderSettings& rs = Fp[sub].render_settings;
                if (has_adaptive_buffers(rs)) {
                    if (rs.sample_number == 0 || rs.need_to_reset) { cnt = 0; f.sq = 0.0f; conv = -1; }
                    bool converged = false;
                    const bool needed = adaptive_gate(rs, f.c, f.sq, cnt, conv, converged);
                    if ((converged || !needed) && rs.do_update_status_buffers) n_conv++;
                    if (!needed) {
                        f.c = f.c / (float)rs.sample_number * (float)(rs.sample_number + 1);
                        continue;
                    }
                    cnt++;
                }
                if (rs.do_update_status_buffers) any = true;
                accumulate_sample(P, rs, batch_slot(P, pixel, sub), f, any);
            }
            P.as_count[pixel] = cnt;
            P.as_conv[pixel] = conv;
        } else {
            for (int sub = 0; sub < P.batch; sub++) accumulate_sample(P, Fp[sub].render_settings, batch_slot(P, pixel, sub), f, any);
        }
        fb[0] = f.c.r; fb[1] = f.c.g; fb[2] = f.c.b;
        fa[0] = f.a.x; fa[1] = f.a.y; fa[2] = f.a.z;
        fn[0] = f.n.x; fn[1] = f.n.y; fn[2] = f.n.z;
        if (adaptive) P.as_sqlum[pixel] = f.sq;
    }
    if (__ballot(any) != 0ull && lane_id() == 0) P.status[1] = 1u;
    if (P.spec_as) {
        for (int off = 32; off > 0; off >>= 1) n_conv += __shfl_xor(n_conv, off);
        if (lane_id() == 0 && n_conv) atomicAdd(&P.status[0], n_conv);
    }
}

#endif
void part_shade_generic(dim3 g, hipStream_t st, const ShadeArgs& a);
void part_shade_plain(dim3 g, hipStream_t st, const ShadeArgs& a);
void part_shade_glass(dim3 g, hipStream_t st, const ShadeArgs& a);
void part_shade_plain_stage(int stage, dim3 g, hipStream_t st, const ShadeArgs& a);
void part_shade_ext(dim3 g, hipStream_t st, const ShadeArgs& a);
void part_shade_override(int ovr, bool ext, dim3 g, hipStream_t st, const ShadeArgs& a);
enum RestirKernel { RK_INITIAL, RK_SPATIOTEMPORAL, RK_SPATIOTEMPORAL_ANY, RK_SPATIAL, RK_SPATIAL_ANY, RK_TEMPORAL, RK_SP_SELECT,
                   RK_SP_EVAL_PLAIN, RK_SP_EVAL_GENERIC, RK_SP_COMBINE, RK_INITIAL_STAGED_PLAIN, RK_INITIAL_STAGED_GENERIC,
                   RK_ST_SELECT, RK_ST_EVAL_PLAIN, RK_ST_EVAL_GENERIC, RK_ST_COMBINE };
void part_restir_principled(int kind, dim3 g, hipStream_t st, const DevScene& S, const DevPaths& P, const MptFrame* F,
                            int pass, const float4* in, float4* out);
void part_restir_override(int ovr, int kind, dim3 g, hipStream_t st, const DevScene& S, const DevPaths& P,
                          const MptFrame* F, int pass, const float4* in, float4* out);
#ifndef MPT_TU_PART
static int blocks_for(int n) { return (n + TB - 1) / TB; }

__global__ void k_count_add64(uint64_t* dst, const int32_t* src) {
    if (threadIdx.x == 0) atomicAdd((unsigned long long*)dst, (unsigned long long)(uint32_t)*src);
}

static void launch_restir_kernel(int ovr, int kind, dim3 g, hipStream_t st, const DevScene& S, const DevPaths& P,
                                 const MptFrame* F, int pass = 0, const float4* in = nullptr, float4* out = nullptr) {
    if (ovr == MPT_BSDF_NONE) part_restir_principled(kind, g, st, S, P, F, pass, in, out);
    else part_restir_override(ovr, kind, g, st, S, P, F, pass, in, out);
}

template <int MODE>
static void launch_trace_mode(const TraceArgs& a, int grid, bool stats, hipStream_t st) {
    if (MODE == TM_NEE_LIGHT && a.static_grid && !stats) grid = blocks_for(a.P.n);
    if (MODE == TM_LIST_ANY || MODE == TM_LIST_CLOSEST) grid = grid / MPT_TRACE_WAVES * MPT_TRACE_WAVES_LIST;
    if (stats) {
        TraceArgs b = a;
        b.static_grid = 0;
        hipLaunchKernelGGL((k_trace<MODE, true>), dim3(grid), dim3(TB), 0, st, b);
    }
    else hipLaunchKernelGGL((k_trace<MODE, false>), dim3(grid), dim3(TB), 0, st, a);
}

struct TimedScope {
    LaunchCfg& cfg;
    hipStream_t st;
    int idx;
    TimedScope(LaunchCfg& c, hipStream_t s, int kind) : cfg(c), st(s), idx(-1) {
        if (c.ev_pool && c.ev_used + 2 <= c.ev_cap) {
            idx = cfg.ev_used;
            cfg.ev_used += 2;
            cfg.ev_mode[idx / 2] = kind;
            hipEventRecord(cfg.ev_pool[idx], st);
        }
    }
    ~TimedScope() {
        if (idx >= 0) hipEventRecord(cfg.ev_pool[idx + 1], st);
    }
};

template <int MODE>
static void timed_trace(const TraceArgs& a, LaunchCfg& cfg, hipStream_t st) {
    bool timed = cfg.ev_pool && cfg.ev_used + 2 <= cfg.ev_cap;
    if (timed) { cfg.ev_mode[cfg.ev_used / 2] = trace_stage(MODE); hipEventRecord(cfg.ev_pool[cfg.ev_used], st); }
    launch_trace_mode<MODE>(a, cfg.grid_persistent, cfg.stats, st);
    if (timed) { hipEventRecord(cfg.ev_pool[cfg.ev_used + 1], st); cfg.ev_used += 2; }
    cfg.launches++;
}

static float4* restir_buffer(const DevPaths& P, int code) { return code == 1 ? P.rs_sp2 : code == 2 ? P.rs_init : P.rs_sp1; }
static int restir_code(const DevPaths& P, const float4* b) { return b == P.rs_sp2 ? 1 : b == P.rs_init ? 2 : 0; }

static int halo_exchange(const MptFrame& hf, LaunchCfg& cfg, hipStream_t st, int phase, int pass, int halo,
                         std::initializer_list<std::pair<void*, int64_t>> bufs, bool agreed = false) {
    if (!cfg.halo_fn || cfg.halo_rc) return halo;
    MptHaloExchange x{};
    x.halo_agreed = agreed ? 1 : 0;
    x.phase = phase;
    x.pass = pass;
    x.res_x = hf.res_x;
    x.res_y = hf.res_y;
    x.own_y0 = cfg.own_y0;
    x.own_y1 = cfg.own_y1;
    x.halo_rows = halo;
    for (const auto& b : bufs) {
        if (!b.first || x.n_buffers >= MPT_HALO_MAX_BUFFERS) continue;
        x.buffers[x.n_buffers] = b.first;
        x.bytes_per_pixel[x.n_buffers] = b.second;
        x.n_buffers++;
    }
// ... 214 lines not shown
        if (rd.do_spatial_reuse_pass) {
            for (int pass = 0; pass < rd.number_of_passes; pass++) {
                float4* in = pass == 0 ? cur : ((pass & 1) ? P.rs_sp1 : P.rs_sp2);
                float4* out = pass == 0 ? P.rs_sp1 : ((pass & 1) ? P.rs_sp2 : P.rs_sp1);
                halo_exchange(hf, cfg, st, MPT_HALO_RESERVOIRS, pass + 1, cfg.halo_rows, {{in, RB}});
                TimedScope tk(cfg, st, KT_RS_SPATIAL);
                launch_spatial_pass(ovr, def_bias, hf, cfg, g, st, S, P, d_frame, pass, in, out);
                cur = out;
            }
        }
        P.rs_out = cur;
    }
    cfg.restir_out_sp2 = restir_code(P, P.rs_out);
}

static void restir_first_bounce(const DevScene& S, DevPaths& P, const MptFrame* d_frame, const MptFrame& hf, LaunchCfg& cfg,
                                hipStream_t st) {
    {
        TimedScope tk(cfg, st, KT_GBUFFER);
        hipLaunchKernelGGL(k_gbuffer, dim3(blocks_for(P.n)), dim3(TB), 0, st, S, P, d_frame);
    }
    launch_restir(S, P, d_frame, hf, cfg, st);
}

static void frame_bounces(const DevScene& S, DevPaths& P, const MptFrame* d_frame, const MptFrame& hf, LaunchCfg& cfg,
                          hipStream_t st, int b_first, int b_last, int32_t* q_cur, int c_cur, int32_t* q_next,
                          int c_next, bool first_traced = false, bool restir_done = false) {
    const int n = P.n;
    const bool restir = hf.options.direct_light_sampling == MPT_LSS_RESTIR_DI;
    const int nb = hf.render_settings.nb_bounces;
    const bool ext = P.x_per > 0;
    const int classes = (hf.options.bsdf_override != MPT_BSDF_NONE || ext) ? 0 : (cfg.shade_classes != 0 ? (cfg.shade_glass ? 2 : 1) : 0);
    const bool ahead = cfg.ahead_stream != nullptr && (!restir || restir_done || b_first > 0);
    const bool pipe = cfg.nee_stream != nullptr && cfg.pipe_alt != nullptr && !restir && !ext && !cfg.shade_split;
    DevPaths PB = P;
    DevPaths* const Pout = &P;
    bool nee_pending = false;
    for (int b = b_first; b <= b_last; b++) {
        DevPaths Pv = (pipe && (b & 1)) ? *cfg.pipe_alt : PB;
        if (pipe) Pv.ce = (b & 1) ? cfg.pipe_alt->ce : PB.ce;
        DevPaths& P = Pv;
        int32_t* const cnt_cur = &PB.counters[c_cur];
        int32_t* const cnt_next = &PB.counters[c_next];
        hipMemsetAsync(&P.counters[CTR_BOUNCE_FIRST], 0, (CTR_COUNT - CTR_BOUNCE_FIRST) * sizeof(int32_t), st);
        const int alpha = hf.render_settings.do_alpha_testing ? 1 : 0;
        if (!(first_traced && b == b_first) && !(ahead && b > b_first)) {
            TraceArgs ta{};
            ta.S = S; ta.P = P; ta.queue = q_cur; ta.count_ptr = cnt_cur; ta.fetch = &P.counters[CTR_F_PATH];
            ta.F = d_frame; ta.bounce = b; ta.alpha = alpha;
            timed_trace<TM_PATH>(ta, cfg, st);
        }
        if (b == 0 && cfg.ev_first_trace) hipEventRecord(cfg.ev_first_trace, st);
        if (restir && b == 0 && !restir_done) {
            restir_first_bounce(S, P, d_frame, hf, cfg, st);
            PB.rs_out = Pout->rs_out = P.rs_out;
        }
        const dim3 cp_grid((n + CP_NT * CP_ITEMS - 1) / (CP_NT * CP_ITEMS));
        {
            TimedScope ts(cfg, st, KT_SPLIT);
            hipLaunchKernelGGL(k_split, cp_grid, dim3(CP_NT), 0, st, S, P, q_cur, cnt_cur, classes, cnt_next);
        }
        ShadeArgs sa{};
        sa.S = S; sa.P = P; sa.F = d_frame; sa.bounce = b; sa.last_bounce = nb;
        sa.q_cur = P.qh; sa.count_cur = &P.counters[CTR_HIT]; sa.q_defer = P.qf; sa.count_defer = &P.counters[CTR_FULL];
        sa.force_defer = cfg.shade_classes == 2 ? 1 : 0;
        sa.mat_private = cfg.mat_private;
        {
            TimedScope ts(cfg, st, KT_SHADE);
            const dim3 sg(blocks_for(n));
            if (hf.options.bsdf_override != MPT_BSDF_NONE) part_shade_override(hf.options.bsdf_override, ext, sg, st, sa);
            else if (ext) part_shade_ext(sg, st, sa);
            else if (!classes) part_shade_generic(sg, st, sa);
            else if (cfg.shade_split) {
                static const int splits[3][3] = {{SG_LIGHT, SG_ENV, SG_CONT}, {SG_LIGHT, SG_ENV | SG_CONT, 0},
                                                 {SG_LIGHT | SG_ENV, SG_CONT, 0}};
                const MptWorldSettings& ws = hf.world_settings;
                const bool env = ws.ambient_light_type == MPT_AMBIENT_ENVMAP && !hf.bsdf_flags.white_furnace_mode &&
                                 ws.envmap_intensity > 0.0f && hf.options.envmap_sampling != MPT_ESS_NO_SAMPLING &&
                                 !(hf.options.direct_light_sampling == MPT_LSS_RESTIR_DI && b == 0);
                const int work = SG_LIGHT | (env ? SG_ENV : 0) | (b < nb ? SG_CONT : 0);
                const int* sp = splits[std::min(std::max(cfg.shade_split, 1), 3) - 1];
                for (int k = 0; k < 3 && sp[k]; k++)
                    if (sp[k] & work) part_shade_plain_stage(sp[k], sg, st, sa);
            } else part_shade_plain(sg, st, sa);
        }
        if (classes) {
            TimedScope ts(cfg, st, KT_SHADE_GENERIC);
            ShadeArgs sf = sa;
            sf.q_cur = P.qf; sf.count_cur = &P.counters[CTR_FULL]; sf.q_defer = nullptr; sf.count_defer = nullptr;
            part_shade_generic(dim3(blocks_for(n)), st, sf);
            if (classes == 2) {
                ShadeArgs sg2 = sf;
                sg2.q_cur = P.qf + P.n; sg2.count_cur = &P.counters[CTR_GLASS]; sg2.rev = 1;
                part_shade_glass(dim3(blocks_for(n)), st, sg2);
            }
        }
        if (nee_pending) { hipStreamWaitEvent(st, cfg.ev_nee_join, 0); nee_pending = false; }
        {
            TimedScope ts(cfg, st, KT_MISS);
            hipLaunchKernelGGL(k_miss, dim3(std::min(blocks_for(n), 8 * cfg.grid_persistent)), dim3(TB), 0, st, S, P, d_frame, b);
        }
        {
            TimedScope ts(cfg, st, KT_COMPACT);
            const dim3 cp_grid2((2 * n + CP_NT * CP_ITEMS - 1) / (CP_NT * CP_ITEMS));
            int32_t* const next_fetch = (pipe && !(b & 1)) ? &cfg.pipe_alt->counters[CTR_F_PATH] : &PB.counters[CTR_F_PATH];
            hipLaunchKernelGGL(k_compact, classes ? cp_grid2 : cp_grid, dim3(CP_NT), 0, st, P, q_next, cnt_next,
                               ahead && b < b_last ? next_fetch : nullptr);
        }
        const bool fork = ahead && b < b_last;
        if (fork) {
            hipEventRecord(cfg.ev_ahead_fork, st);
            hipStreamWaitEvent(cfg.ahead_stream, cfg.ev_ahead_fork, 0);
            DevPaths PA = (pipe && !(b & 1)) ? *cfg.pipe_alt : PB;
            PA.stack_spill = cfg.ahead_spill;
            TraceArgs ta{};
            ta.S = S; ta.P = PA; ta.queue = q_next; ta.count_ptr = cnt_next; ta.fetch = &PA.counters[CTR_F_PATH];
            ta.F = d_frame; ta.bounce = b + 1; ta.alpha = hf.render_settings.do_alpha_testing ? 1 : 0;
            timed_trace<TM_PATH>(ta, cfg, cfg.ahead_stream);
            hipEventRecord(cfg.ev_ahead_join, cfg.ahead_stream);
            cfg.ahead_launches++;
        }
        const hipStream_t main_st = st;
        if (pipe) {
            hipEventRecord(cfg.ev_nee_fork, main_st);
            hipStreamWaitEvent(cfg.nee_stream, cfg.ev_nee_fork, 0);
            st = cfg.nee_stream;
            P.stack_spill = cfg.nee_spill;
        }
        TraceArgs tn{};
        tn.S = S; tn.P = P; tn.count_ptr = &P.counters[CTR_ANY]; tn.fetch = &P.counters[CTR_F_ANY];
        tn.F = d_frame; tn.bounce = b; tn.alpha = alpha;
        timed_trace<TM_NEE_ANY>(tn, cfg, st);
        tn.fetch = &P.counters[CTR_F_CL];
        tn.count_ptr = &P.counters[CTR_CL];
        if (cfg.light_bvh) {
            tn.static_grid = cfg.light_static;
            timed_trace<TM_NEE_LIGHT>(tn, cfg, st);
            tn.static_grid = 0;
            tn.fetch = &P.counters[CTR_F_OCC];
            tn.count_ptr = &P.counters[CTR_LIGHT];
            timed_trace<TM_NEE_LIGHT_OCC>(tn, cfg, st);
        } else {
            timed_trace<TM_NEE_CLOSEST>(tn, cfg, st);
        }
        if (ext) {
            TraceArgs tx = tn;
            tx.ext = 1;
            tx.static_grid = 0;
            tx.fetch = &P.counters[CTR_F_XANY];
            tx.count_ptr = &P.counters[CTR_XANY];
            timed_trace<TM_NEE_ANY>(tx, cfg, st);
            tx.fetch = &P.counters[CTR_F_XCL];
            tx.count_ptr = &P.counters[CTR_XCL];
            if (cfg.light_bvh) {
                timed_trace<TM_NEE_LIGHT>(tx, cfg, st);
                tx.fetch = &P.counters[CTR_F_XOCC];
                tx.count_ptr = &P.counters[CTR_XLIGHT];
                timed_trace<TM_NEE_LIGHT_OCC>(tx, cfg, st);
            } else {
                timed_trace<TM_NEE_CLOSEST>(tx, cfg, st);
            }
        }
        {
            TimedScope ts(cfg, st, KT_RESOLVE);
            const dim3 rg(std::min(blocks_for(classes ? 2 * n : n), 8 * cfg.grid_persistent));
            if (ext) hipLaunchKernelGGL(k_resolve<true>, rg, dim3(TB), 0, st, S, P, d_frame, b, cnt_cur);
            else hipLaunchKernelGGL(k_resolve<false>, rg, dim3(TB), 0, st, S, P, d_frame, b, cnt_cur);
// ... 331 lines not shown
```

hiprt-path-tracer_amd/csrc/mpt_part.hip:

```cpp
#ifndef MPT_TU_PART
#error "compile with -DMPT_TU_PART=<1..7>"
#endif
#include "mpt_kernels.hip"

namespace mpt {

#if MPT_TU_PART == 1
void part_shade_generic(dim3 g, hipStream_t st, const ShadeArgs& a) {
    if (a.mat_private) hipLaunchKernelGGL((k_shade<MPT_BSDF_NONE, false, false, false, SG_ALL, true>), g, dim3(TB), 0, st, a);
    else hipLaunchKernelGGL((k_shade<MPT_BSDF_NONE, false>), g, dim3(TB), 0, st, a);
}
#elif MPT_TU_PART == 2
void part_shade_plain(dim3 g, hipStream_t st, const ShadeArgs& a) {
    if (a.mat_private) hipLaunchKernelGGL((k_shade<MPT_BSDF_NONE, true, false, false, SG_ALL, true>), g, dim3(TB), 0, st, a);
    else hipLaunchKernelGGL((k_shade<MPT_BSDF_NONE, true>), g, dim3(TB), 0, st, a);
}
#ifdef MPT_SECTION_TIMING
extern "C" int mpt_debug_sections(unsigned long long* out, int reset) {
    hipMemcpyFromSymbol(out, HIP_SYMBOL(g_sect), sizeof(unsigned long long) * 8);
    if (reset) { unsigned long long z[8] = {0}; hipMemcpyToSymbol(HIP_SYMBOL(g_sect), z, sizeof(z)); }
    return 0;
}
#endif
#elif MPT_TU_PART == 7
void part_shade_plain_stage(int stage, dim3 g, hipStream_t st, const ShadeArgs& a) {
    switch (stage) {
    case SG_LIGHT: hipLaunchKernelGGL((k_shade<MPT_BSDF_NONE, true, false, false, SG_LIGHT>), g, dim3(TB), 0, st, a); break;
    case SG_ENV: hipLaunchKernelGGL((k_shade<MPT_BSDF_NONE, true, false, false, SG_ENV>), g, dim3(TB), 0, st, a); break;
    case SG_CONT: hipLaunchKernelGGL((k_shade<MPT_BSDF_NONE, true, false, false, SG_CONT>), g, dim3(TB), 0, st, a); break;
    case SG_LIGHT | SG_ENV:
        hipLaunchKernelGGL((k_shade<MPT_BSDF_NONE, true, false, false, SG_LIGHT | SG_ENV>), g, dim3(TB), 0, st, a);
        break;
    default: hipLaunchKernelGGL((k_shade<MPT_BSDF_NONE, true, false, false, SG_ENV | SG_CONT>), g, dim3(TB), 0, st, a); break;
    }
}
#elif MPT_TU_PART == 3
void part_shade_ext(dim3 g, hipStream_t st, const ShadeArgs& a) {
    hipLaunchKernelGGL((k_shade<MPT_BSDF_NONE, false, true>), g, dim3(TB), 0, st, a);
}
void part_shade_glass(dim3 g, hipStream_t st, const ShadeArgs& a) {
    hipLaunchKernelGGL((k_shade<MPT_BSDF_NONE, false, false, true>), g, dim3(TB), 0, st, a);
}
#elif MPT_TU_PART == 4
void part_shade_override(int ovr, bool ext, dim3 g, hipStream_t st, const ShadeArgs& a) {
    if (ovr == MPT_BSDF_LAMBERTIAN) {
        if (ext) hipLaunchKernelGGL((k_shade<MPT_BSDF_LAMBERTIAN, false, true>), g, dim3(TB), 0, st, a);
        else hipLaunchKernelGGL((k_shade<MPT_BSDF_LAMBERTIAN, false>), g, dim3(TB), 0, st, a);
    } else {
        if (ext) hipLaunchKernelGGL((k_shade<MPT_BSDF_OREN_NAYAR, false, true>), g, dim3(TB), 0, st, a);
        else hipLaunchKernelGGL((k_shade<MPT_BSDF_OREN_NAYAR, false>), g, dim3(TB), 0, st, a);
    }
}
#elif MPT_TU_PART == 5 || MPT_TU_PART == 6
template <int OVR>
static void restir_kernel(int kind, dim3 g, hipStream_t st, const DevScene& S, const DevPaths& P, const MptFrame* F, int pass,
                          const float4* in, float4* out) {
    constexpr int DEF = MPT_RESTIR_DI_BIAS_PAIRWISE_MIS_DEFENSIVE;
    switch (kind) {
    case RK_INITIAL: hipLaunchKernelGGL((k_restir_initial<OVR, false>), g, dim3(TB), 0, st, S, P, F, nullptr, nullptr); break;
    case RK_INITIAL_STAGED_PLAIN:
        if (OVR == MPT_BSDF_NONE)
            hipLaunchKernelGGL((k_restir_initial<OVR, true, true>), g, dim3(TB), 0, st, S, P, F, P.rq_items, &P.counters[CTR_RQE0]);
        break;
    case RK_INITIAL_STAGED_GENERIC:
        hipLaunchKernelGGL((k_restir_initial<OVR, true, false>), g, dim3(TB), 0, st, S, P, F, P.rq_items + P.n,
                           &P.counters[CTR_RQE1]);
        break;
    case RK_SPATIOTEMPORAL: hipLaunchKernelGGL((k_restir_spatiotemporal<OVR, DEF>), g, dim3(TB), 0, st, S, P, F); break;
    case RK_SPATIOTEMPORAL_ANY: hipLaunchKernelGGL((k_restir_spatiotemporal<OVR, -1>), g, dim3(TB), 0, st, S, P, F); break;
    case RK_SPATIAL:
        hipLaunchKernelGGL((k_restir_spatial<OVR, DEF>), g, dim3(TB), 0, st, S, P, F, pass, in, out);
        break;
    case RK_SPATIAL_ANY:
        hipLaunchKernelGGL((k_restir_spatial<OVR, -1>), g, dim3(TB), 0, st, S, P, F, pass, in, out);
        break;
    case RK_SP_SELECT: hipLaunchKernelGGL(k_rsp_select<OVR>, g, dim3(TB), 0, st, S, P, F, pass, in); break;
    case RK_SP_EVAL_PLAIN:
        if (OVR == MPT_BSDF_NONE)
            hipLaunchKernelGGL((k_rsp_eval<OVR, true, false>), g, dim3(TB), 0, st, S, P, F, pass, in, P.rq_items, &P.counters[CTR_RQE0]);
        break;
    case RK_SP_EVAL_GENERIC:
        hipLaunchKernelGGL((k_rsp_eval<OVR, false, false>), g, dim3(TB), 0, st, S, P, F, pass, in, P.rq_items + (size_t)P.n * RS_RPP,
                           &P.counters[CTR_RQE1]);
        break;
    case RK_ST_SELECT: hipLaunchKernelGGL(k_rst_select<OVR>, g, dim3(TB), 0, st, S, P, F); break;
    case RK_ST_EVAL_PLAIN:
        if (OVR == MPT_BSDF_NONE)
            hipLaunchKernelGGL((k_rsp_eval<OVR, true, true>), g, dim3(TB), 0, st, S, P, F, 0, P.rs_tin, P.rq_items,
                               &P.counters[CTR_RQE0]);
        break;
    case RK_ST_EVAL_GENERIC:
        hipLaunchKernelGGL((k_rsp_eval<OVR, false, true>), g, dim3(TB), 0, st, S, P, F, 0, P.rs_tin,
                           P.rq_items + (size_t)P.n * RS_RPP, &P.counters[CTR_RQE1]);
        break;
    case RK_ST_COMBINE: hipLaunchKernelGGL(k_rst_combine<OVR>, g, dim3(TB), 0, st, S, P, F); break;
    case RK_SP_COMBINE: hipLaunchKernelGGL(k_rsp_combine<OVR>, g, dim3(TB), 0, st, S, P, F, pass, in, out); break;
    default: hipLaunchKernelGGL(k_restir_temporal<OVR>, g, dim3(TB), 0, st, S, P, F, in, out); break;
    }
}
#if MPT_TU_PART == 5
void part_restir_principled(int kind, dim3 g, hipStream_t st, const DevScene& S, const DevPaths& P, const MptFrame* F, int pass,
                            const float4* in, float4* out) {
    restir_kernel<MPT_BSDF_NONE>(kind, g, st, S, P, F, pass, in, out);
}
#else
// ... 10 lines not shown
```

hiprt-path-tracer_amd/mpt/__init__.py:

```python
from __future__ import annotations

import ctypes as C
import os

import numpy as np

from . import abi
from . import scene
from ._build import LIB_PATH

__all__ = ["abi", "scene", "lib", "GPURenderer", "MptError", "build_envmap", "partition_rows", "display_settings",
           "display_host", "write_png", "denoise_host", "bvh_refit_host", "bvh_build_host"]

SYMBOLS = [
    "mpt_last_error", "mpt_version", "mpt_abi_sizes", "mpt_create", "mpt_destroy", "mpt_upload_scene",
    "mpt_update_materials", "mpt_set_envmap", "mpt_build_alias_table", "mpt_set_luts", "mpt_resize",
    "mpt_render_frame", "mpt_render_frames", "mpt_synchronize", "mpt_query_done", "mpt_get_framebuffer", "mpt_partition_rows",
    "mpt_enable_stats", "mpt_get_stats", "mpt_trace_closest", "mpt_trace_any", "mpt_clear_status",
    "mpt_query_status", "mpt_get_aux_buffer", "mpt_build_envmap_cdf", "mpt_set_envmap_cdf", "mpt_set_halo_exchange",
    "mpt_set_halo_native", "mpt_halo_plan", "mpt_set_pipeline",
    "mpt_bake_lut", "mpt_png_unfilter", "mpt_device_info", "mpt_gather", "mpt_comm_unique_id", "mpt_comm_init",
    "mpt_comm_gather", "mpt_jpeg_decode", "mpt_hdr_decode",
    "mpt_display_settings_default", "mpt_display_uniforms", "mpt_display", "mpt_display_host", "mpt_write_png",
    "mpt_denoise_settings_default", "mpt_denoise", "mpt_denoised_buffer", "mpt_denoise_device", "mpt_denoise_host",
    "mpt_update_vertices", "mpt_get_bvh", "mpt_bvh_refit_host", "mpt_rebuild_bvh", "mpt_bvh_build_host",
    "mpt_rebuild_bvh_mode", "mpt_bvh_build_host_mode",
]


class MptError(RuntimeError):
    def __init__(self, code, msg):
        super().__init__(f"mpt error {code}: {msg}")
        self.code = code


_lib = None


def lib() -> C.CDLL:
    global _lib
    if _lib is not None:
        return _lib
    path = os.environ.get("MPT_LIB_PATH", str(LIB_PATH))
    if not os.path.exists(path):
        raise ImportError(f"libmpt.so not found at {path}; run __graft_entry__.build() (no CPU fallback)")
    try:
        import torch
    except ImportError:
        pass
    L = C.CDLL(path)
    vp, i32, f32 = C.c_void_p, C.c_int32, C.c_float
    L.mpt_last_error.restype = C.c_char_p
    L.mpt_abi_sizes.argtypes = [vp, C.c_int]
    L.mpt_create.argtypes = [C.c_int, vp, C.POINTER(vp)]
    L.mpt_destroy.argtypes = [vp]
    L.mpt_upload_scene.argtypes = [vp, C.POINTER(abi.Scene)]
    L.mpt_update_materials.argtypes = [vp, vp, i32]
    L.mpt_set_envmap.argtypes = [vp, vp, i32, i32, vp, vp, f32]
    L.mpt_build_alias_table.argtypes = [vp, i32, i32, vp, vp, vp]
    L.mpt_set_luts.argtypes = [vp, C.POINTER(abi.Luts)]
    L.mpt_resize.argtypes = [vp, i32, i32]
    L.mpt_render_frame.argtypes = [vp, C.POINTER(abi.Frame)]
    L.mpt_render_frames.argtypes = [vp, C.POINTER(abi.Frame), i32, i32]
    L.mpt_synchronize.argtypes = [vp]
    L.mpt_query_done.argtypes = [vp, C.POINTER(C.c_int)]
    L.mpt_get_framebuffer.argtypes = [vp, C.c_int, vp, C.c_int]
    L.mpt_partition_rows.argtypes = [i32, i32, i32, i32]
    L.mpt_enable_stats.argtypes = [vp, C.c_int, C.c_int]
    L.mpt_get_stats.argtypes = [vp, C.POINTER(abi.Stats)]
    L.mpt_trace_closest.argtypes = [vp, vp, vp, i32, vp, vp, vp, vp, C.c_int]
    L.mpt_trace_any.argtypes = [vp, vp, vp, i32, vp, C.c_int]
    L.mpt_png_unfilter.argtypes = [vp, C.c_int64, vp, i32, i32, i32]
    L.mpt_device_info.argtypes = [C.c_int, vp, i32, vp, i32, vp]
    L.mpt_build_envmap_cdf.argtypes = [vp, i32, i32, vp, vp]
    L.mpt_set_envmap_cdf.argtypes = [vp, vp, f32]
    L.mpt_clear_status.argtypes = [vp]
    L.mpt_query_status.argtypes = [vp, C.POINTER(abi.Status)]
    L.mpt_get_aux_buffer.argtypes = [vp, C.c_int, vp, C.c_int]
    L.mpt_set_halo_exchange.argtypes = [vp, abi.HaloExchangeFn, vp]
    L.mpt_set_halo_native.argtypes = [vp, C.c_int32]
    L.mpt_set_pipeline.argtypes = [vp, C.c_int32]
    L.mpt_halo_plan.argtypes = [i32, i32, i32, i32, i32, i32, C.POINTER(abi.HaloOp), i32]
    L.mpt_bake_lut.argtypes = [vp, C.c_int, i32, i32, i32, i32, vp, C.c_int]
    L.mpt_gather.argtypes = [C.POINTER(vp), i32, i32, C.c_int, vp, C.c_int]
    L.mpt_comm_unique_id.argtypes = [vp, i32]
    L.mpt_comm_init.argtypes = [vp, i32, i32, vp]
    L.mpt_comm_gather.argtypes = [vp, i32, C.c_int, vp, C.c_int]
    L.mpt_jpeg_decode.argtypes = [vp, C.c_int64, i32, vp, C.c_int64, vp, vp, vp]
    L.mpt_hdr_decode.argtypes = [vp, C.c_int64, i32, vp, C.c_int64, vp, vp]
    L.mpt_display_settings_default.argtypes = [C.POINTER(abi.DisplaySettings)]
    L.mpt_display_uniforms.argtypes = [C.POINTER(abi.RenderSettings), i32, i32, C.POINTER(abi.DisplaySettings)]
    L.mpt_display.argtypes = [vp, C.POINTER(abi.DisplaySettings), vp, C.c_int, vp, C.c_int]
    L.mpt_display_host.argtypes = [C.POINTER(abi.DisplaySettings), vp, vp, i32, i32, vp]
    L.mpt_write_png.argtypes = [C.c_char_p, vp, i32, i32, i32]
    L.mpt_denoise_settings_default.argtypes = [C.POINTER(abi.DenoiseSettings)]
    L.mpt_denoise.argtypes = [vp, C.POINTER(abi.DenoiseSettings), vp, C.c_int]
    L.mpt_denoised_buffer.argtypes = [vp, C.POINTER(vp), C.POINTER(i32)]
    L.mpt_denoise_device.argtypes = [vp, C.POINTER(abi.DenoiseSettings), vp, vp, vp, i32, i32, vp]
    L.mpt_denoise_host.argtypes = [C.POINTER(abi.DenoiseSettings), vp, vp, vp, i32, i32, vp]
    L.mpt_update_vertices.argtypes = [vp, vp, vp, i32, C.POINTER(abi.RefitInfo)]
    L.mpt_get_bvh.argtypes = [vp, C.c_int, vp, C.c_int64, vp, C.c_int64, vp]
    L.mpt_bvh_refit_host.argtypes = [vp, vp, i32, vp, i32, vp, C.c_int64, vp, C.c_int64, vp]
    L.mpt_rebuild_bvh.argtypes = [vp, C.POINTER(abi.RebuildInfo)]
    L.mpt_bvh_build_host.argtypes = [vp, i32, vp, i32, vp, i32, vp, C.c_int64, vp, C.c_int64, vp]
    L.mpt_rebuild_bvh_mode.argtypes = [vp, i32, C.POINTER(abi.RebuildInfo)]
    L.mpt_bvh_build_host_mode.argtypes = [vp, i32, vp, i32, vp, i32, i32, vp, C.c_int64, vp, C.c_int64, vp]
    _lib = L
    return L


def _check(rc):
    if rc != 0:
        raise MptError(rc, lib().mpt_last_error().decode(errors="replace"))


def _p(a):
    return None if a is None else C.c_void_p(a.ctypes.data)


def abi_sizes():
    out = np.zeros(8, np.int32)
    _check(lib().mpt_abi_sizes(_p(out), 8))
    sizes = dict(zip(["Material", "RenderSettings", "WorldSettings", "Camera", "Frame", "Scene", "Stats",
                      "DisplaySettings"], out.tolist()))
    if sizes["DisplaySettings"] != C.sizeof(abi.DisplaySettings):
        raise MptError(abi.ERR_INVALID_ARGUMENT, f"MptDisplaySettings is {sizes['DisplaySettings']} bytes in libmpt.so, "
                       f"{C.sizeof(abi.DisplaySettings)} in mpt.abi")
    return sizes


def device_info(device=0):
    name, arch, cus = C.create_string_buffer(256), C.create_string_buffer(64), C.c_int32()
    _check(lib().mpt_device_info(device, name, 256, arch, 64, C.byref(cus)))
    return name.value.decode(errors="replace"), arch.value.decode(errors="replace"), int(cus.value)


def build_id():
    import hashlib
    return hashlib.sha256(open(lib()._name, "rb").read()).hexdigest()[:16]


def partition_rows(res_y, band_height, band_index, band_count):
    return lib().mpt_partition_rows(res_y, band_height, band_index, band_count)


def halo_plan(res_y, band_height, band_count, band_index, halo_rows, n_buffers=1):
    args = (res_y, band_height, band_count, band_index, halo_rows, n_buffers)
    n = lib().mpt_halo_plan(*args, None, 0)
    _check(min(n, 0))
    ops = (abi.HaloOp * max(n, 1))()
    m = lib().mpt_halo_plan(*args, ops, n)
    _check(min(m, 0))
    return [(o.peer, "recv" if o.recv else "send", o.buffer, o.row_lo, o.row_hi) for o in ops[:m]]


GATHER_AUX = 16


def _gather_out(f, kind):
    if kind >= GATHER_AUX:
        return np.zeros((f.res_y, f.res_x), np.float32 if kind == GATHER_AUX + abi.AUX_SQUARED_LUMINANCE else np.int32)
    return np.zeros((f.res_y, f.res_x, 3), np.float32)


# ... 107 lines not shown
class GPURenderer:

    def __init__(self, device: int = 0, stream: int | None = None):
        L = lib()
        h = C.c_void_p()
        _check(L.mpt_create(device, C.c_void_p(stream) if stream else None, C.byref(h)))
        self.h = h
        self.device = device
        self.frame = None
        self._n_mats = 0

    def set_scene(self, sd: "scene.SceneData"):
        s = sd.to_abi()
        _check(lib().mpt_upload_scene(self.h, C.byref(s)))
        self._n_mats = len(sd.materials)

    def update_materials(self, materials):
        arr = (abi.Material * len(materials))(*materials)
        _check(lib().mpt_update_materials(self.h, C.cast(arr, C.c_void_p), len(materials)))

    def update_vertices(self, vertices, normals=None, info=False):
        v = np.ascontiguousarray(vertices, np.float32).reshape(-1, 3)
        n = None
        if normals is not None:
            n = np.ascontiguousarray(normals, np.float32).reshape(-1, 3)
            if n.shape != v.shape:
                raise ValueError(f"update_vertices: {n.shape[0]} normals for {v.shape[0]} vertices")
        ri = abi.RefitInfo() if info else None
        _check(lib().mpt_update_vertices(self.h, _p(v), _p(n), v.shape[0], C.byref(ri) if info else None))
        return ri

    def rebuild_bvh(self, info=False, mode=abi.BUILD_LBVH):
        ri = abi.RebuildInfo() if info else None
        _check(lib().mpt_rebuild_bvh_mode(self.h, int(mode), C.byref(ri) if info else None))
        return ri

    def get_bvh(self, which=0):
        L = lib()
        return _bvh_arrays(lambda n, nc, t, tc, cnt: L.mpt_get_bvh(self.h, which, n, nc, t, tc, cnt))

    def set_envmap(self, env):
        if env is None:
            _check(lib().mpt_set_envmap(self.h, None, 0, 0, None, None, 0.0))
            return
        self._env = env
        _check(lib().mpt_set_envmap(self.h, _p(env["rgba"]), env["width"], env["height"], _p(env["probas"]),
                                    _p(env["alias"]), env["sum"]))
        if env.get("cdf") is not None:
            _check(lib().mpt_set_envmap_cdf(self.h, _p(env["cdf"]), env["cdf_sum"]))

    def set_luts(self, luts=None):
        luts = luts if luts is not None else scene.load_luts()
        L = scene.luts_to_abi(luts)
        _check(lib().mpt_set_luts(self.h, C.byref(L)))

    def resize(self, w, h):
        _check(lib().mpt_resize(self.h, w, h))

    def set_halo_exchange(self, exchange):
        if exchange is None:
            self._halo_cb = None
            _check(lib().mpt_set_halo_exchange(self.h, abi.HaloExchangeFn(), None))
            return

        def _cb(_user, xp):
            try:
                exchange(xp.contents)
                return 0
            except BaseException as e:
                self._halo_error = e
                return 1

        self._halo_error = None
        self._halo_cb = abi.HaloExchangeFn(_cb)
        _check(lib().mpt_set_halo_exchange(self.h, self._halo_cb, None))

    def set_halo_native(self, mode: int):
        self._halo_cb = None
        _check(lib().mpt_set_halo_native(self.h, int(mode)))

    def set_pipeline(self, mode: int):
        _check(lib().mpt_set_pipeline(self.h, int(mode)))

    def render(self, frame: "abi.Frame"):
        rc = lib().mpt_render_frame(self.h, C.byref(frame))
        err = getattr(self, "_halo_error", None)
        if err is not None:
            self._halo_error = None
            raise MptError(rc or -1, f"halo exchange failed: {err!r}") from err
        _check(rc)
        self.frame = frame

    def render_samples(self, frames, max_batch: int = 0):
        if not frames:
            return
        arr = (abi.Frame * len(frames))(*frames)
        rc = lib().mpt_render_frames(self.h, arr, len(frames), int(max_batch))
        err = getattr(self, "_halo_error", None)
        if err is not None:
            self._halo_error = None
            raise MptError(rc or -1, f"halo exchange failed: {err!r}") from err
        _check(rc)
        self.frame = frames[-1]

    def synchronize_kernel(self):
        _check(lib().mpt_synchronize(self.h))

    def frame_render_done(self) -> bool:
        d = C.c_int()
        _check(lib().mpt_query_done(self.h, C.byref(d)))
        return bool(d.value)

    def rows(self):
        f = self.frame
        return partition_rows(f.res_y, f.band_height, f.band_index, f.band_count)

    def framebuffer(self, kind=abi.FB_COLOR):
        f = self.frame
        out = np.zeros((self.rows(), f.res_x, 3), np.float32)
        _check(lib().mpt_get_framebuffer(self.h, kind, _p(out), 0))
        return out

    def framebuffer_to_device(self, kind, dev_ptr: int):
        _check(lib().mpt_get_framebuffer(self.h, kind, C.c_void_p(dev_ptr), 1))

    def display_settings(self, view=abi.VIEW_DEFAULT, low_resolution=False, base=None):
        if self.frame is None:
            raise MptError(abi.ERR_INVALID_ARGUMENT, "display: no frame rendered")
        rs = abi.RenderSettings.from_buffer_copy(self.frame.render_settings)
        rs.sample_number += 1
        return display_settings(rs, view, low_resolution, base)

    def _display(self, view, settings, second, second_is_device, low_resolution, dst, dst_is_device):
        s = settings if settings is not None else self.display_settings(view, low_resolution)
        _check(lib().mpt_display(self.h, C.byref(s), second, int(second_is_device), dst, int(dst_is_device)))

    def display(self, view=abi.VIEW_DEFAULT, settings=None, second=None, low_resolution=False):
        out = np.zeros((self.rows(), self.frame.res_x, 4), np.uint8)
        if isinstance(second, (int, np.integer)):
            sec, dev = C.c_void_p(int(second)), True
        else:
            second = None if second is None else np.ascontiguousarray(second, np.float32)
            if second is not None and second.size != 3 * out.shape[0] * out.shape[1]:
                raise ValueError(f"display: second buffer of shape {second.shape}")
            sec, dev = _p(second), False
        self._display(view, settings, sec, dev, low_resolution, _p(out), False)
        return out

    def display_to_device(self, dev_ptr: int, view=abi.VIEW_DEFAULT, settings=None, second_dev_ptr: int | None = None,
                          low_resolution=False):
        sec = C.c_void_p(int(second_dev_ptr)) if second_dev_ptr else None
        self._display(view, settings, sec, True, low_resolution, C.c_void_p(int(dev_ptr)), True)

    def denoise_settings(self, base=None):
        if self.frame is None:
            raise MptError(abi.ERR_INVALID_ARGUMENT, "denoise: no frame rendered")
        s = abi.DenoiseSettings.default()
        if base is not None:
            C.memmove(C.byref(s), C.byref(base), C.sizeof(s))
        s.sample_number = self.frame.render_settings.sample_number + 1
        return s

    def denoise(self, settings=None):
        s = settings if settings is not None else self.denoise_settings()
        if self.frame is None:
            raise MptError(abi.ERR_INVALID_ARGUMENT, "denoise: no frame rendered")
# ... 98 lines not shown
```

hiprt-path-tracer_amd/mpt/_build.py:

```python
from __future__ import annotations

import os
import subprocess
import sys
from pathlib import Path

PKG_DIR = Path(__file__).resolve().parent
ROOT = PKG_DIR.parent
CSRC = ROOT / "csrc"
INCLUDE = ROOT.parent / "include"
LIB_PATH = PKG_DIR / "libmpt.so"
OBJ_DIR = CSRC / "build"

SOURCES = ["bvh8.cpp", "mpt_kernels.hip", "bake.hip", "mpt_api.cpp", "image.cpp", "jpeg.cpp", "display.hip", "denoise.hip", "refit.hip", "lbvh.hip", "ploc.hip", "sah.hip"]
PARTS = [1, 2, 3, 4, 5, 6, 7]
HIPCC = os.environ.get("HIPCC", "/opt/rocm/bin/hipcc")
ARCH = "gfx950"
CXXFLAGS = [
    f"--offload-arch={ARCH}", "-O3", "-std=c++17", "-fPIC", "-ffp-contract=off",
    "-Wno-unused-result", "-Wno-unused-value", f"-I{INCLUDE}", f"-I{CSRC}",
]


def _deps() -> list[Path]:
    return [CSRC / s for s in SOURCES] + [CSRC / "mpt_part.hip"] + sorted(CSRC.glob("*.h")) + sorted(INCLUDE.glob("*.h"))


def up_to_date() -> bool:
    if not LIB_PATH.exists():
        return False
    t = LIB_PATH.stat().st_mtime
    return all(p.stat().st_mtime <= t for p in _deps())


def build(force: bool = False, verbose: bool = True, defines=(), out: Path | None = None) -> Path:
    lib_path = Path(out) if out else LIB_PATH
    if not force and not defines and out is None and up_to_date():
        return LIB_PATH
    obj_dir = OBJ_DIR if out is None else lib_path.parent / "obj"
    obj_dir.mkdir(parents=True, exist_ok=True)
    procs = []
    objs = []
    units = [(s, [], Path(s).stem) for s in SOURCES] + [("mpt_part.hip", [f"-DMPT_TU_PART={k}"], f"mpt_part{k}") for k in PARTS]
    for s, extra, stem in units:
        obj = obj_dir / (stem + ".o")
        objs.append(obj)
        cmd = [HIPCC, *CXXFLAGS, *defines, *extra, "-c", str(CSRC / s), "-o", str(obj)]
        if verbose:
            print("[mpt build]", " ".join(cmd), file=sys.stderr)
        procs.append((stem, subprocess.Popen(cmd, stdout=subprocess.PIPE, stderr=subprocess.STDOUT)))
    errors = []
    for s, p in procs:
        out, _ = p.communicate()
        if p.returncode != 0:
            errors.append(f"{s}:\n{out.decode(errors='replace')}")
    if errors:
        raise RuntimeError("libmpt build failed:\n" + "\n".join(errors))
    tmp = lib_path.with_suffix(".so.tmp")
    cmd = [HIPCC, f"--offload-arch={ARCH}", "-shared", "-fPIC", "-o", str(tmp), *map(str, objs)]
    r = subprocess.run(cmd, stdout=subprocess.PIPE, stderr=subprocess.STDOUT)
    if r.returncode != 0:
        raise RuntimeError("libmpt link failed:\n" + r.stdout.decode(errors="replace"))
    os.replace(tmp, lib_path)
    return lib_path


HOST_DIR = ROOT / "host"
HOST_TEST = HOST_DIR / "gpurenderer_parity"
HOST_SOURCES = [HOST_DIR / "gpu_renderer.cpp", ROOT.parent / "tests" / "cpp" / "gpurenderer_parity.cpp"]
DISPLAY_TEST = HOST_DIR / "display_views"
DISPLAY_SOURCES = [HOST_DIR / "gpu_renderer.cpp", ROOT.parent / "tests" / "cpp" / "display_views.cpp"]
DENOISE_TEST = HOST_DIR / "denoise_blend"
DENOISE_SOURCES = [HOST_DIR / "gpu_renderer.cpp", ROOT.parent / "tests" / "cpp" / "denoise_blend.cpp"]
REFIT_TEST = HOST_DIR / "refit_move"
REFIT_SOURCES = [HOST_DIR / "gpu_renderer.cpp", ROOT.parent / "tests" / "cpp" / "refit_move.cpp"]
REBUILD_TEST = HOST_DIR / "rebuild_move"
REBUILD_SOURCES = [HOST_DIR / "gpu_renderer.cpp", ROOT.parent / "tests" / "cpp" / "rebuild_move.cpp"]
PLOC_TEST = HOST_DIR / "ploc_move"
PLOC_SOURCES = [HOST_DIR / "gpu_renderer.cpp", ROOT.parent / "tests" / "cpp" / "ploc_move.cpp"]


def _build_driver(exe: Path, sources, lib: Path, verbose: bool) -> Path:
    deps = list(sources) + sorted(HOST_DIR.glob("*.h")) + [lib]
    if exe.exists() and all(p.stat().st_mtime <= exe.stat().st_mtime for p in deps):
        return exe
    cmd = ["g++", "-O2", "-std=c++17", "-D__HIP_PLATFORM_AMD__", f"-I{INCLUDE}", f"-I{HOST_DIR}", "-I/opt/rocm/include",
           *map(str, sources), f"-L{PKG_DIR}", "-lmpt", "-L/opt/rocm/lib", "-lamdhip64",
           "-Wl,-rpath,$ORIGIN/../mpt", "-Wl,-rpath,/opt/rocm/lib",
           "-Wl,-rpath-link,/opt/rocm/lib", "-o", str(exe)]
    if verbose:
        print("[mpt build]", " ".join(cmd), file=sys.stderr)
    r = subprocess.run(cmd, stdout=subprocess.PIPE, stderr=subprocess.STDOUT)
    if r.returncode != 0:
        raise RuntimeError("host test build failed:\n" + r.stdout.decode(errors="replace"))
    return exe


def build_host_test(verbose: bool = True) -> Path:
# ... 15 lines not shown
```

include/mpt.h:

```cpp
#ifndef MPT_H
#define MPT_H

#include <stddef.h>
#include <stdint.h>
#include <stdbool.h>

#ifdef __cplusplus
extern "C" {
#endif

#define MPT_OK 0
#define MPT_ERR_INVALID_ARGUMENT (-1)
#define MPT_ERR_HIP (-2)
#define MPT_ERR_NO_SCENE (-3)
#define MPT_ERR_UNSUPPORTED (-4)
#define MPT_ERR_OUT_OF_MEMORY (-5)

#define MPT_BSDF_NONE 0
#define MPT_BSDF_LAMBERTIAN 1
#define MPT_BSDF_OREN_NAYAR 2

#define MPT_LSS_NO_DIRECT_LIGHT_SAMPLING 0
#define MPT_LSS_UNIFORM_ONE_LIGHT 1
#define MPT_LSS_BSDF 2
// ... 327 lines not shown

typedef struct MptContext MptContext;

#define MPT_HALO_GBUFFER 0
#define MPT_HALO_RESERVOIRS 1
#define MPT_HALO_PREV_GBUFFER 2
#define MPT_HALO_MAX_BUFFERS 12
typedef struct MptHaloExchange {
    int32_t phase;
    int32_t pass;
    int32_t res_x, res_y;
    int32_t own_y0, own_y1;
    int32_t halo_rows;
    int32_t n_buffers;
    void* buffers[MPT_HALO_MAX_BUFFERS];
    int64_t bytes_per_pixel[MPT_HALO_MAX_BUFFERS];
    void* stream;
    int32_t halo_agreed;
} MptHaloExchange;
typedef int (*MptHaloExchangeFn)(void* user, MptHaloExchange* x);

const char* mpt_last_error(void);
int mpt_version(void);
int mpt_abi_sizes(int32_t* out_sizes, int n);
int mpt_device_info(int device, char* name, int32_t name_cap, char* arch, int32_t arch_cap, int32_t* out_cus);

int mpt_create(int device, void* hip_stream, MptContext** out_ctx);
int mpt_destroy(MptContext* ctx);
int mpt_upload_scene(MptContext* ctx, const MptScene* scene);
int mpt_update_materials(MptContext* ctx, const MptMaterial* materials, int32_t count);

typedef struct MptRefitInfo {
    int32_t nodes, levels, light_nodes, light_levels;
    float area_ratio, light_area_ratio;
} MptRefitInfo;
int mpt_update_vertices(MptContext* ctx, const float* vertices, const float* vertex_normals_or_NULL,
                        int32_t num_vertices, MptRefitInfo* info_or_NULL);
int mpt_get_bvh(MptContext* ctx, int which, void* nodes, int64_t nodes_cap_bytes, void* tris, int64_t tris_cap_bytes,
                int32_t* out_counts);
int mpt_bvh_refit_host(const float* build_vertices, const float* new_vertices_or_NULL, int32_t num_vertices,
                       const int32_t* indices, int32_t num_triangles, void* nodes, int64_t nodes_cap_bytes,
                       void* tris, int64_t tris_cap_bytes, int32_t* out_counts);
typedef struct MptRebuildInfo {
    int32_t rebuilt, nodes, records, levels;
    int32_t light_rebuilt, light_nodes, light_records, light_levels;
} MptRebuildInfo;
int mpt_rebuild_bvh(MptContext* ctx, MptRebuildInfo* info_or_NULL);
#define MPT_BUILD_LBVH 0
#define MPT_BUILD_PLOC 1
#define MPT_BUILD_SAH 3
int mpt_rebuild_bvh_mode(MptContext* ctx, int32_t mode, MptRebuildInfo* info_or_NULL);
int mpt_bvh_build_host(const float* vertices, int32_t num_vertices, const int32_t* indices, int32_t num_triangles,
                       const int32_t* prims_or_NULL, int32_t num_prims, void* nodes, int64_t nodes_cap_bytes, void* tris,
                       int64_t tris_cap_bytes, int32_t* out_counts);
int mpt_bvh_build_host_mode(const float* vertices, int32_t num_vertices, const int32_t* indices, int32_t num_triangles,
                            const int32_t* prims_or_NULL, int32_t num_prims, int32_t mode, void* nodes,
                            int64_t nodes_cap_bytes, void* tris, int64_t tris_cap_bytes, int32_t* out_counts);
int mpt_set_envmap(MptContext* ctx, const float* rgba, int32_t width, int32_t height,
                   const float* alias_probas, const int32_t* alias_indices, float luminance_total_sum);
int mpt_build_alias_table(const float* rgba, int32_t width, int32_t height,
                          float* out_probas, int32_t* out_alias, float* out_luminance_sum);
int mpt_build_envmap_cdf(const float* rgba, int32_t width, int32_t height, float* out_cdf, float* out_total_sum);
int mpt_set_envmap_cdf(MptContext* ctx, const float* cdf, float total_sum);
int mpt_set_luts(MptContext* ctx, const MptLuts* luts);
int mpt_resize(MptContext* ctx, int32_t width, int32_t height);
int mpt_render_frame(MptContext* ctx, const MptFrame* frame);
#define MPT_MAX_BATCH 128
#define MPT_DEFAULT_WAVEFRONT_PATHS (1 << 25)
#define MPT_MAX_WAVEFRONT_PATHS (1 << 29)
int mpt_render_frames(MptContext* ctx, const MptFrame* frames, int32_t count, int32_t max_batch);
int mpt_set_halo_exchange(MptContext* ctx, MptHaloExchangeFn fn, void* user);
int mpt_synchronize(MptContext* ctx);
int mpt_query_done(MptContext* ctx, int* out_done);
int mpt_get_framebuffer(MptContext* ctx, int kind, float* dst, int dst_is_device);
int mpt_partition_rows(int32_t res_y, int32_t band_height, int32_t band_index, int32_t band_count);
#define MPT_GATHER_AUX 16
int mpt_gather(MptContext* const* ctxs, int32_t n, int32_t root, int kind, void* dst, int dst_is_device);
#define MPT_COMM_ID_BYTES 128
int mpt_comm_unique_id(uint8_t* out_id, int32_t cap);
int mpt_comm_init(MptContext* ctx, int32_t nranks, int32_t rank, const uint8_t* id);
int mpt_comm_gather(MptContext* ctx, int32_t root, int kind, void* dst, int dst_is_device);
int mpt_set_halo_native(MptContext* ctx, int32_t mode);
int mpt_set_pipeline(MptContext* ctx, int32_t mode);
typedef struct MptHaloOp {
    int32_t peer;
    int32_t recv;
    int32_t buffer;
    int32_t row_lo, row_hi;
} MptHaloOp;
int mpt_halo_plan(int32_t res_y, int32_t band_height, int32_t band_count, int32_t band_index, int32_t halo_rows,
                  int32_t n_buffers, MptHaloOp* out, int32_t cap);
int mpt_clear_status(MptContext* ctx);
int mpt_query_status(MptContext* ctx, MptStatus* out);
int mpt_get_aux_buffer(MptContext* ctx, int kind, void* dst, int dst_is_device);
int mpt_enable_stats(MptContext* ctx, int enable, int instrumented);
int mpt_get_stats(MptContext* ctx, MptStats* out);
#define MPT_BAKE_GGX_CONDUCTOR 0
#define MPT_BAKE_GGX_FRESNEL 1
#define MPT_BAKE_GLOSSY_DIELECTRIC 2
#define MPT_BAKE_GGX_GLASS 3
#define MPT_BAKE_GGX_GLASS_INVERSE 4
#define MPT_BAKE_GGX_THIN_GLASS 5
int mpt_bake_lut(MptContext* ctx, int kind, int32_t width, int32_t height, int32_t depth, int32_t sample_count,
                 float* out, int out_is_device);
int mpt_trace_closest(MptContext* ctx, const float* rays, const int32_t* last_hit, int32_t n,
                      int32_t* out_prim, float* out_t, float* out_u, float* out_v, int pointers_are_device);
int mpt_trace_any(MptContext* ctx, const float* rays, const int32_t* last_hit, int32_t n,
                  uint8_t* out_occluded, int pointers_are_device);

int mpt_png_unfilter(const uint8_t* filtered, int64_t filtered_size, uint8_t* out, int32_t rows, int32_t row_bytes,
                     int32_t bpp);
int mpt_jpeg_decode(const uint8_t* data, int64_t size, int32_t req_comp, uint8_t* out, int64_t out_cap,
                    int32_t* out_w, int32_t* out_h, int32_t* out_comp);
int mpt_hdr_decode(const uint8_t* data, int64_t size, int32_t req_comp, float* out, int64_t out_cap,
                   int32_t* out_w, int32_t* out_h);

#define MPT_VIEW_DEFAULT 0
#define MPT_VIEW_BLEND 1
#define MPT_VIEW_NORMALS 2
#define MPT_VIEW_ALBEDO 4
#define MPT_VIEW_PIXEL_CONVERGENCE_HEATMAP 6
#define MPT_VIEW_PIXEL_CONVERGED_MAP 7
#define MPT_VIEW_WHITE_FURNACE_THRESHOLD 8
#define MPT_DISPLAY_MAX_STOPS 16

typedef struct MptDisplaySettings {
    int32_t view;
    int32_t sample_number;
    int32_t sample_number_2;
    int32_t resolution_scaling;
    int32_t do_tonemapping;
    float gamma;
    float exposure;
    float blend_factor;
    int32_t use_low_threshold;
    int32_t use_high_threshold;
    float min_val;
    float max_val;
    float threshold_val;
    int32_t nb_stops;
    MptColor color_stops[MPT_DISPLAY_MAX_STOPS];
} MptDisplaySettings;

int mpt_display_settings_default(MptDisplaySettings* out);
int mpt_display_uniforms(const MptRenderSettings* render_settings, int32_t view, int32_t low_resolution_displayed,
                         MptDisplaySettings* inout);
int mpt_display(MptContext* ctx, const MptDisplaySettings* settings, const float* second_rgb, int second_is_device,
                uint8_t* dst_rgba8, int dst_is_device);
int mpt_display_host(const MptDisplaySettings* settings, const void* src, const float* src2, int32_t width,
                     int32_t height, uint8_t* dst_rgba8);
int mpt_write_png(const char* path, const uint8_t* rgba8, int32_t width, int32_t height, int32_t flip_y);

#define MPT_DENOISE_MAX_ITERATIONS 8
typedef struct MptDenoiseSettings {
    int32_t sample_number;
    int32_t iterations;
    int32_t use_albedo;
    int32_t use_normals;
    float sigma_color;
    float sigma_albedo;
    int32_t normal_power_log2;
} MptDenoiseSettings;

int mpt_denoise_settings_default(MptDenoiseSettings* out);
int mpt_denoise(MptContext* ctx, const MptDenoiseSettings* settings, float* dst_rgb_or_NULL, int dst_is_device);
int mpt_denoised_buffer(MptContext* ctx, const float** dev, int32_t* sample_number);
// ... 11 lines not shown
```

Measured before the change: 3550.

## Specialise plain shade kernel per sampling plan to prune dead op branches

Adds compile-time sampling plans (RIS with env, RIS, MIS, ReSTIR bounce 0) chosen on the host per bounce, and launches a plain shade kernel instantiation for each plan that compiles out the sampling ops the plan never uses. It also reloads the vertex throughput and previous colour late instead of keeping them live, which lowers register pressure, and gives the plan kernels their own waves-per-EU targets. The intent is smaller kernels with fewer registers and higher occupancy. The cost is four extra translation units and a larger binary, and the host-side plan choice must agree with the device logic.

Result: no change. 3560, median of 6 (+0.3%).

```diff
diff --git a/hiprt-path-tracer_amd/csrc/mpt_api.cpp b/hiprt-path-tracer_amd/csrc/mpt_api.cpp
--- a/hiprt-path-tracer_amd/csrc/mpt_api.cpp
+++ b/hiprt-path-tracer_amd/csrc/mpt_api.cpp
@@ -155,6 +155,7 @@
     int adaptive_batch = 1;
     int restir_max_batch = RESTIR_MAX_BATCH;
     int shade_glass = 1;
+    int shade_plans = 1;
     int shade_split = 0;
     int shade_texmetal = 1;
     std::vector<MptMaterial> h_mats;
@@ -940,6 +941,7 @@
     if (const char* e = std::getenv("MPT_RESTIR_CHUNK")) c->restir_chunk = std::atoi(e);
     if (const char* e = std::getenv("MPT_SHADE_GLASS")) c->shade_glass = std::atoi(e);
     if (const char* e = std::getenv("MPT_SHADE_SPLIT")) c->shade_split = std::atoi(e);
+    if (const char* e = std::getenv("MPT_SHADE_PLANS")) c->shade_plans = std::atoi(e) != 0;
     if (const char* e = std::getenv("MPT_SHADE_TEXMETAL")) c->shade_texmetal = std::atoi(e);
     if (const char* e = std::getenv("MPT_LIGHT_BVH")) c->light_bvh = std::atoi(e);
     if (const char* e = std::getenv("MPT_OVERLAP")) c->overlap = std::atoi(e);
@@ -1543,8 +1545,8 @@
     k.render_settings.denoiser_AOV_accumulation_counter = 0;
     k.render_settings.need_to_reset = false;
     k.render_settings.do_update_status_buffers = false;
-    const int flags[9] = {cfg.grid_persistent, cfg.stats, cfg.shade_classes, cfg.light_bvh, cfg.light_static,
-                          cfg.restir_staged, cfg.shade_glass, cfg.shade_split, cfg.mat_private};
+    const int flags[10] = {cfg.grid_persistent, cfg.stats, cfg.shade_classes, cfg.light_bvh, cfg.light_static,
+                           cfg.restir_staged, cfg.shade_glass, cfg.shade_split, cfg.mat_private, cfg.shade_plans};
     std::vector<uint8_t> key(sizeof(k) + sizeof(S) + sizeof(P) + sizeof(flags));
     uint8_t* q = key.data();
     std::memcpy(q, &k, sizeof(k)); q += sizeof(k);
@@ -1729,6 +1731,7 @@
     }
     cfg.shade_glass = c->shade_glass && c->any_glass;
     cfg.shade_split = c->shade_split;
+    cfg.shade_plans = c->shade_plans;
     cfg.mat_private = c->mat_private >= 0 ? (c->mat_private != 0) : (c->tex_tri_frac >= 0.25);
     cfg.light_bvh = c->light_bvh && c->light_bvh_ok;
     cfg.light_static = !c->h_light_prims.empty() && 2 * c->bvh_light.depth + 2 <= TRAV_LDS_STACK;
@@ -2454,6 +2457,23 @@
     return MPT_OK;
 }
 
+int mpt_set_shade_plans(MptContext* c, int32_t mode) {
+    if (!c) return fail(MPT_ERR_INVALID_ARGUMENT, "NULL context");
+    if (mode < 0 || mode > 1) return fail(MPT_ERR_INVALID_ARGUMENT, "mode must be 0 (generic plain kernel) or 1 (by sampling plan)");
+    c->shade_plans = mode;
+    return MPT_OK;
+}
+
+int mpt_debug_shade_plan(const MptFrame* f, int32_t bounce, int32_t scene_has_emissives) {
+    if (!f || bounce < 0) return fail(MPT_ERR_INVALID_ARGUMENT, "mpt_debug_shade_plan: NULL frame or negative bounce");
+    return shade_plan(*f, bounce, scene_has_emissives);
+}
+
+int mpt_debug_shade_plan_ops(int32_t plan) {
+    if (plan < 0 || plan >= SP_COUNT) return fail(MPT_ERR_INVALID_ARGUMENT, "mpt_debug_shade_plan_ops: no such plan");
+    return (int)shade_plan_ops(plan);
+}
+
 int mpt_set_halo_native(MptContext* c, int32_t mode) {
     if (!c) return fail(MPT_ERR_INVALID_ARGUMENT, "NULL context");
     if (mode < 0 || mode > 2) return fail(MPT_ERR_INVALID_ARGUMENT, "mode must be 0 (off), 1 (RCCL) or 2 (rehearsal)");
diff --git a/hiprt-path-tracer_amd/csrc/mpt_internal.h b/hiprt-path-tracer_amd/csrc/mpt_internal.h
--- a/hiprt-path-tracer_amd/csrc/mpt_internal.h
+++ b/hiprt-path-tracer_amd/csrc/mpt_internal.h
@@ -208,6 +208,43 @@
 constexpr int STATS_STRIDE = 6;
 constexpr int N_STATS = N_TRACE_MODES * STATS_STRIDE;
 
+enum ShadeOp {
+    OP_DONE = 0, OP_RIS_LIGHT, OP_RIS_BSDF, OP_RIS_WIN, OP_MIS_LIGHT, OP_MIS_BSDF, OP_UNI_LIGHT, OP_BSDF_LIGHT,
+    OP_ENV_LIGHT, OP_ENV_BSDF, OP_CONT, OP_RESTIR
+};
+enum ShadePlan { SP_GENERIC = 0, SP_RIS_ENV = 1, SP_RIS = 2, SP_MIS = 3, SP_RESTIR0 = 4, SP_COUNT = 5 };
+constexpr uint32_t OPS_RIS = 1u << OP_RIS_LIGHT | 1u << OP_RIS_BSDF | 1u << OP_RIS_WIN;
+constexpr uint32_t OPS_ENV = 1u << OP_ENV_LIGHT | 1u << OP_ENV_BSDF;
+constexpr uint32_t shade_plan_ops(int plan) {
+    return plan == SP_RIS_ENV ? (OPS_RIS | OPS_ENV | 1u << OP_CONT)
+           : plan == SP_RIS   ? (OPS_RIS | 1u << OP_CONT)
+           : plan == SP_MIS   ? (1u << OP_MIS_LIGHT | 1u << OP_MIS_BSDF | 1u << OP_CONT)
+           : plan == SP_RESTIR0 ? (1u << OP_RESTIR | 1u << OP_CONT)
+                                : 0xffeu;
+}
+inline int frame_bounce_lss(const MptFrame& F, int bounce) {
+    const int lss = F.options.direct_light_sampling;
+    if (lss != MPT_LSS_RESTIR_DI || bounce == 0) return lss;
+    switch (F.options.restir_di_later_bounces_sampling_strategy) {
+    case MPT_RESTIR_DI_LATER_BOUNCES_UNIFORM_ONE_LIGHT: return MPT_LSS_UNIFORM_ONE_LIGHT;
+    case MPT_RESTIR_DI_LATER_BOUNCES_BSDF: return MPT_LSS_BSDF;
+    case MPT_RESTIR_DI_LATER_BOUNCES_MIS_LIGHT_BSDF: return MPT_LSS_MIS_LIGHT_BSDF;
+    default: return MPT_LSS_RIS_BSDF_AND_LIGHT;
+    }
+}
+inline int shade_plan(const MptFrame& F, int bounce, int has_emissives) {
+    (void)has_emissives;
+    const MptWorldSettings& ws = F.world_settings;
+    const bool restir0 = F.options.direct_light_sampling == MPT_LSS_RESTIR_DI && bounce == 0;
+    if (restir0) return SP_RESTIR0;
+    const bool env = ws.ambient_light_type == MPT_AMBIENT_ENVMAP && !F.bsdf_flags.white_furnace_mode &&
+                     ws.envmap_intensity > 0.0f && F.options.envmap_sampling != MPT_ESS_NO_SAMPLING;
+    const int lssb = frame_bounce_lss(F, bounce);
+    if (lssb == MPT_LSS_RIS_BSDF_AND_LIGHT) return env ? SP_RIS_ENV : SP_RIS;
+    if (lssb == MPT_LSS_MIS_LIGHT_BSDF && !env) return SP_MIS;
+    return SP_GENERIC;
+}
+
 enum {
     CTR_Q0 = 0, CTR_Q1 = 1,
     CTR_QG = 2,
@@ -252,6 +289,7 @@
     int restir_mono_reuse;
     int shade_glass;
     int mat_private;
+    int shade_plans;
     int shade_split;
     hipEvent_t ev_first_trace;
     hipEvent_t ev_acc_done;
diff --git a/hiprt-path-tracer_amd/csrc/mpt_kernels.hip b/hiprt-path-tracer_amd/csrc/mpt_kernels.hip
--- a/hiprt-path-tracer_amd/csrc/mpt_kernels.hip
+++ b/hiprt-path-tracer_amd/csrc/mpt_kernels.hip
@@ -1240,10 +1240,6 @@
     return clamp_contrib(sky * thr, rs.indirect_contribution_clamp, bounce > 0);
 }
 
-enum ShadeOp {
-    OP_DONE = 0, OP_RIS_LIGHT, OP_RIS_BSDF, OP_RIS_WIN, OP_MIS_LIGHT, OP_MIS_BSDF, OP_UNI_LIGHT, OP_BSDF_LIGHT,
-    OP_ENV_LIGHT, OP_ENV_BSDF, OP_CONT, OP_RESTIR
-};
 enum { SG_LIGHT = 1, SG_ENV = 2, SG_CONT = 4, SG_ALL = 7 };
 DEV constexpr int op_group(int op) {
     return op == OP_DONE ? 0 : (op == OP_ENV_LIGHT || op == OP_ENV_BSDF) ? SG_ENV : op == OP_CONT ? SG_CONT : SG_LIGHT;
@@ -1283,18 +1279,32 @@
 #ifndef MPT_SHADE_WAVES_PLAIN
 #define MPT_SHADE_WAVES_PLAIN MPT_SHADE_WAVES
 #endif
-#define OPIS(X) ((ST & op_group(X)) && op == (X))
+#define OPIS(X) ((ST & op_group(X)) && (shade_plan_ops(PLAN) >> (X) & 1u) && op == (X))
+#ifndef MPT_SHADE_PEP_PLAN
+#define MPT_SHADE_PEP_PLAN 1
+#endif
+#ifndef MPT_SHADE_WAVES_PLAN_ENV
+#define MPT_SHADE_WAVES_PLAN_ENV 3
+#endif
+#ifndef MPT_SHADE_WAVES_PLAN
+#define MPT_SHADE_WAVES_PLAN 3
+#endif
+DEV constexpr int plan_waves(int plan) {
+    return plan == SP_GENERIC ? MPT_SHADE_WAVES_PLAIN : plan == SP_RIS_ENV ? MPT_SHADE_WAVES_PLAN_ENV
+           : plan == SP_RESTIR0 ? (MPT_SHADE_WAVES_PLAN < 2 ? MPT_SHADE_WAVES_PLAN : 2) : MPT_SHADE_WAVES_PLAN;
+}
 #ifndef MPT_SHADE_WAVES_LATE
 #define MPT_SHADE_WAVES_LATE 3
 #endif
 #ifndef MPT_SHADE_PE_LDS_LATE
 #define MPT_SHADE_PE_LDS_LATE 0
 #endif
-template <int OVR, bool PLAIN, bool EXT = false, bool GLASS = false, int ST = SG_ALL, bool MATP = false>
+template <int OVR, bool PLAIN, bool EXT = false, bool GLASS = false, int ST = SG_ALL, bool MATP = false, int PLAN = SP_GENERIC>
 __global__ __launch_bounds__(TB) __attribute__((amdgpu_waves_per_eu(
-    !(ST & SG_LIGHT) ? MPT_SHADE_WAVES_LATE : (PLAIN ? MPT_SHADE_WAVES_PLAIN : MPT_SHADE_WAVES)))) void k_shade(ShadeArgs A) {
+    !(ST & SG_LIGHT) ? MPT_SHADE_WAVES_LATE : (PLAIN ? plan_waves(PLAN) : MPT_SHADE_WAVES)))) void k_shade(ShadeArgs A) {
+    static_assert(PLAN == SP_GENERIC || (PLAIN && ST == SG_ALL && !EXT && OVR == MPT_BSDF_NONE), "sampling plans: the plain kernel in one stage");
     constexpr int CLS = PLAIN ? BC_PLAIN : (GLASS ? BC_GLASS : BC_FULL);
-    constexpr bool PE_PLAIN = MPT_SHADE_PEP && PLAIN && OVR == MPT_BSDF_NONE && !EXT;
+    constexpr bool PE_PLAIN = (PLAN != SP_GENERIC ? MPT_SHADE_PEP_PLAN : MPT_SHADE_PEP) && PLAIN && OVR == MPT_BSDF_NONE && !EXT;
     constexpr bool FIRST = (ST & SG_LIGHT) != 0;
     constexpr bool LAST = (ST & SG_CONT) != 0;
     static_assert(!EXT || ST == SG_ALL, "extended light sampling shades in one stage");
@@ -1327,12 +1337,16 @@
         Rng rng = make_rng(ld_s(&P.rng[slot]));
         const float4 thv = ld_s(&P.thr[slot]);
         Col thr = col(thv.x, thv.y, thv.z);
-        const Col thr_vertex = thr;
-        Col rcol = col(0.0f);
-        if (!P.ce) {
+        const auto thr_vertex = [&]() {
+            const float4 t4 = ld_s(&P.thr[slot]);
+            return col(t4.x, t4.y, t4.z);
+        };
+        const auto col_before = [&]() {
+            if (P.ce) return col(0.0f);
             const float4 cv = ld_s(&P.col[slot]);
-            rcol = col(cv.x, cv.y, cv.z);
-        }
+            return col(cv.x, cv.y, cv.z);
+        };
+        Col rcol;
         v3 ip = mk3(0, 0, 0), gn = mk3(0, 0, 0), sn = mk3(0, 0, 0);
         const Mat* mp = S.mats_res;
         bool mat_in_slot = false;
@@ -1408,7 +1422,9 @@
             if (FIRST) fl |= NF_SHADED;
             const int lss = F.options.direct_light_sampling;
             const MptWorldSettings& ws = F.world_settings;
-            const bool restir = lss == MPT_LSS_RESTIR_DI;
+            const bool restir = PLAN == SP_RESTIR0 || lss == MPT_LSS_RESTIR_DI;
+            const bool restir0 = PLAN == SP_GENERIC ? (restir && bounce == 0) : PLAN == SP_RESTIR0;
+            const bool no_direct = PLAN == SP_GENERIC && lss == MPT_LSS_NO_DIRECT_LIGHT_SAMPLING;
             bool do_light = (S.n_emissive != 0 || (restir && ws.ambient_light_type == MPT_AMBIENT_ENVMAP)) &&
                             !(F.bsdf_flags.white_furnace_mode && F.bsdf_flags.white_furnace_mode_turn_off_emissives);
             if (do_light && is_emissive(m)) {
@@ -1419,21 +1435,22 @@
                     st_s(&P.na[slot], make_float4(e.r, e.g, e.b, 0.0f));
                 }
             }
-            do_light = do_light && lss != MPT_LSS_NO_DIRECT_LIGHT_SAMPLING;
-            const int lssb = bounce_lss(F, bounce);
-            if (restir && bounce > 0 && S.n_emissive == 0 && lssb == MPT_LSS_RIS_BSDF_AND_LIGHT) do_light = false;
+            do_light = do_light && !no_direct;
+            const int lssb = (PLAN == SP_RIS_ENV || PLAN == SP_RIS) ? (int)MPT_LSS_RIS_BSDF_AND_LIGHT
+                             : PLAN == SP_MIS ? (int)MPT_LSS_MIS_LIGHT_BSDF : bounce_lss(F, bounce);
+            if (restir && !restir0 && S.n_emissive == 0 && lssb == MPT_LSS_RIS_BSDF_AND_LIGHT) do_light = false;
             if (FIRST && do_light) fl |= NF_L;
-            const bool do_env = ws.ambient_light_type == MPT_AMBIENT_ENVMAP && !F.bsdf_flags.white_furnace_mode &&
-                                !is_emissive(m) && ws.envmap_intensity > 0.0f && F.options.envmap_sampling != MPT_ESS_NO_SAMPLING &&
-                                !(restir && bounce == 0);
-            const bool env_use = lss != MPT_LSS_NO_DIRECT_LIGHT_SAMPLING;
+            const bool do_env = (shade_plan_ops(PLAN) >> OP_ENV_LIGHT & 1u) && ws.ambient_light_type == MPT_AMBIENT_ENVMAP &&
+                                !F.bsdf_flags.white_furnace_mode && !is_emissive(m) && ws.envmap_intensity > 0.0f &&
+                                F.options.envmap_sampling != MPT_ESS_NO_SAMPLING && !restir0;
+            const bool env_use = !no_direct;
             const bool do_cont = bounce < A.last_bounce;
             const float ism = dot(view, gn) < 0 ? -1.0f : 1.0f;
             const v3 ep = ip + sn * 1.0e-4f * ism;
             const int nl = rs.ris_number_of_light_candidates, nbc = rs.ris_number_of_bsdf_candidates;
             int op = OP_DONE;
             if (do_light) {
-                if (restir && bounce == 0) op = OP_RESTIR;
+                if (restir0) op = OP_RESTIR;
                 else if (lssb == MPT_LSS_RIS_BSDF_AND_LIGHT) op = nl > 0 ? OP_RIS_LIGHT : (nbc > 0 ? OP_RIS_BSDF : OP_RIS_WIN);
                 else if (lssb == MPT_LSS_MIS_LIGHT_BSDF) op = OP_MIS_LIGHT;
                 else if (lssb == MPT_LSS_UNIFORM_ONE_LIGHT) op = OP_UNI_LIGHT;
@@ -1458,7 +1475,7 @@
             bsdf_eval_pre<OVR, CLS>(bc, m, vs, view, sn, pe);
             SECT(5);
             if constexpr (EXT) {
-                if (do_light && !(restir && bounce == 0)) {
+                if (do_light && !restir0) {
                     ext_light<OVR, CLS>(S, P, F, bc, m, vs, pe, slot, prim, ip, sn, gn, view, ism, ep, lssb, rng);
                     fl |= NF_EXT;
                     op = do_env ? OP_ENV_LIGHT : (do_cont ? OP_CONT : OP_DONE);
@@ -1711,9 +1728,10 @@
                 op = next < 0 ? OP_DONE : stage_op<ST>(next, do_env, do_cont);
                 SECT(3);
             }
-            if (FIRST && lss == MPT_LSS_NO_DIRECT_LIGHT_SAMPLING) {
+            rcol = col_before();
+            if (FIRST && no_direct) {
                 Col he = clamp_contrib(emission_of(m), rs.indirect_contribution_clamp, bounce > 0);
-                rcol += he * thr_vertex;
+                rcol += he * thr_vertex();
                 fl &= ~(NF_A | NF_B | NF_E1 | NF_E2 | NF_RIS_W | NF_IMM | NF_L);
                 fl |= NF_NOADD;
             } else if (FIRST && bounce == 0) {
@@ -1725,11 +1743,13 @@
                 st_s(&P.s_gn[slot], make_float4(gn.x, gn.y, gn.z, 0.0f));
             }
         } else {
+            rcol = col_before();
             rcol += miss_radiance(S, F, bounce, d, thr);
         }
         const uint32_t qb = qm | (cont ? QM_CONT : 0u);
         if (FIRST) {
-            st_s(&P.nthr[slot], make_float4(thr_vertex.r, thr_vertex.g, thr_vertex.b, __uint_as_float(fl)));
+            const Col tvx = thr_vertex();
+            st_s(&P.nthr[slot], make_float4(tvx.r, tvx.g, tvx.b, __uint_as_float(fl)));
             st_s(&P.qmask[slot], (uint8_t)qb);
             st_s(P.ce ? &P.ce[slot] : &P.col[slot], make_float4(rcol.r, rcol.g, rcol.b, 0.0f));
         } else {
@@ -2261,6 +2281,10 @@
 #endif
 void part_shade_generic(dim3 g, hipStream_t st, const ShadeArgs& a);
 void part_shade_plain(dim3 g, hipStream_t st, const ShadeArgs& a);
+void part_shade_plan_ris_env(dim3 g, hipStream_t st, const ShadeArgs& a);
+void part_shade_plan_ris(dim3 g, hipStream_t st, const ShadeArgs& a);
+void part_shade_plan_mis(dim3 g, hipStream_t st, const ShadeArgs& a);
+void part_shade_plan_restir0(dim3 g, hipStream_t st, const ShadeArgs& a);
 void part_shade_glass(dim3 g, hipStream_t st, const ShadeArgs& a);
 void part_shade_plain_stage(int stage, dim3 g, hipStream_t st, const ShadeArgs& a);
 void part_shade_ext(dim3 g, hipStream_t st, const ShadeArgs& a);
@@ -2641,7 +2665,15 @@
                 const int* sp = splits[std::min(std::max(cfg.shade_split, 1), 3) - 1];
                 for (int k = 0; k < 3 && sp[k]; k++)
                     if (sp[k] & work) part_shade_plain_stage(sp[k], sg, st, sa);
-            } else part_shade_plain(sg, st, sa);
+            } else {
+                switch (cfg.shade_plans ? shade_plan(hf, b, S.n_emissive != 0) : (int)SP_GENERIC) {
+                case SP_RIS_ENV: part_shade_plan_ris_env(sg, st, sa); break;
+                case SP_RIS: part_shade_plan_ris(sg, st, sa); break;
+                case SP_MIS: part_shade_plan_mis(sg, st, sa); break;
+                case SP_RESTIR0: part_shade_plan_restir0(sg, st, sa); break;
+                default: part_shade_plain(sg, st, sa); break;
+                }
+            }
         }
         if (classes) {
             TimedScope ts(cfg, st, KT_SHADE_GENERIC);
diff --git a/hiprt-path-tracer_amd/csrc/mpt_part.hip b/hiprt-path-tracer_amd/csrc/mpt_part.hip
--- a/hiprt-path-tracer_amd/csrc/mpt_part.hip
+++ b/hiprt-path-tracer_amd/csrc/mpt_part.hip
@@ -1,5 +1,5 @@
 #ifndef MPT_TU_PART
-#error "compile with -DMPT_TU_PART=<1..7>"
+#error "compile with -DMPT_TU_PART=<1..11>"
 #endif
 #include "mpt_kernels.hip"
 
@@ -21,6 +21,21 @@
     if (reset) { unsigned long long z[8] = {0}; hipMemcpyToSymbol(HIP_SYMBOL(g_sect), z, sizeof(z)); }
     return 0;
 }
+#endif
+#elif MPT_TU_PART >= 8 && MPT_TU_PART <= 11
+template <int PLAN>
+static void shade_plan_kernel(dim3 g, hipStream_t st, const ShadeArgs& a) {
+    if (a.mat_private) hipLaunchKernelGGL((k_shade<MPT_BSDF_NONE, true, false, false, SG_ALL, true, PLAN>), g, dim3(TB), 0, st, a);
+    else hipLaunchKernelGGL((k_shade<MPT_BSDF_NONE, true, false, false, SG_ALL, false, PLAN>), g, dim3(TB), 0, st, a);
+}
+#if MPT_TU_PART == 8
+void part_shade_plan_ris_env(dim3 g, hipStream_t st, const ShadeArgs& a) { shade_plan_kernel<SP_RIS_ENV>(g, st, a); }
+#elif MPT_TU_PART == 9
+void part_shade_plan_ris(dim3 g, hipStream_t st, const ShadeArgs& a) { shade_plan_kernel<SP_RIS>(g, st, a); }
+#elif MPT_TU_PART == 10
+void part_shade_plan_mis(dim3 g, hipStream_t st, const ShadeArgs& a) { shade_plan_kernel<SP_MIS>(g, st, a); }
+#else
+void part_shade_plan_restir0(dim3 g, hipStream_t st, const ShadeArgs& a) { shade_plan_kernel<SP_RESTIR0>(g, st, a); }
 #endif
 #elif MPT_TU_PART == 7
 void part_shade_plain_stage(int stage, dim3 g, hipStream_t st, const ShadeArgs& a) {
diff --git a/hiprt-path-tracer_amd/mpt/__init__.py b/hiprt-path-tracer_amd/mpt/__init__.py
--- a/hiprt-path-tracer_amd/mpt/__init__.py
+++ b/hiprt-path-tracer_amd/mpt/__init__.py
@@ -18,7 +18,8 @@
     "mpt_render_frame", "mpt_render_frames", "mpt_synchronize", "mpt_query_done", "mpt_get_framebuffer", "mpt_partition_rows",
     "mpt_enable_stats", "mpt_get_stats", "mpt_trace_closest", "mpt_trace_any", "mpt_clear_status",
     "mpt_query_status", "mpt_get_aux_buffer", "mpt_build_envmap_cdf", "mpt_set_envmap_cdf", "mpt_set_halo_exchange",
-    "mpt_set_halo_native", "mpt_halo_plan", "mpt_set_pipeline",
+    "mpt_set_halo_native", "mpt_halo_plan", "mpt_set_pipeline", "mpt_set_shade_plans", "mpt_debug_shade_plan",
+    "mpt_debug_shade_plan_ops",
     "mpt_bake_lut", "mpt_png_unfilter", "mpt_device_info", "mpt_gather", "mpt_comm_unique_id", "mpt_comm_init",
     "mpt_comm_gather", "mpt_jpeg_decode", "mpt_hdr_decode",
     "mpt_display_settings_default", "mpt_display_uniforms", "mpt_display", "mpt_display_host", "mpt_write_png",
@@ -80,6 +81,9 @@
     L.mpt_set_halo_exchange.argtypes = [vp, abi.HaloExchangeFn, vp]
     L.mpt_set_halo_native.argtypes = [vp, C.c_int32]
     L.mpt_set_pipeline.argtypes = [vp, C.c_int32]
+    L.mpt_set_shade_plans.argtypes = [vp, C.c_int32]
+    L.mpt_debug_shade_plan.argtypes = [C.POINTER(abi.Frame), i32, i32]
+    L.mpt_debug_shade_plan_ops.argtypes = [i32]
     L.mpt_halo_plan.argtypes = [i32, i32, i32, i32, i32, i32, C.POINTER(abi.HaloOp), i32]
     L.mpt_bake_lut.argtypes = [vp, C.c_int, i32, i32, i32, i32, vp, C.c_int]
     L.mpt_gather.argtypes = [C.POINTER(vp), i32, i32, C.c_int, vp, C.c_int]
@@ -353,6 +357,9 @@
     def set_pipeline(self, mode: int):
         _check(lib().mpt_set_pipeline(self.h, int(mode)))
 
+    def set_shade_plans(self, mode: int):
+        _check(lib().mpt_set_shade_plans(self.h, int(mode)))
+
     def render(self, frame: "abi.Frame"):
         rc = lib().mpt_render_frame(self.h, C.byref(frame))
         err = getattr(self, "_halo_error", None)
diff --git a/hiprt-path-tracer_amd/mpt/_build.py b/hiprt-path-tracer_amd/mpt/_build.py
--- a/hiprt-path-tracer_amd/mpt/_build.py
+++ b/hiprt-path-tracer_amd/mpt/_build.py
@@ -13,7 +13,7 @@
 OBJ_DIR = CSRC / "build"
 
 SOURCES = ["bvh8.cpp", "mpt_kernels.hip", "bake.hip", "mpt_api.cpp", "image.cpp", "jpeg.cpp", "display.hip", "denoise.hip", "refit.hip", "lbvh.hip", "ploc.hip", "sah.hip"]
-PARTS = [1, 2, 3, 4, 5, 6, 7]
+PARTS = [1, 2, 3, 4, 5, 6, 7, 8, 9, 10, 11]
 HIPCC = os.environ.get("HIPCC", "/opt/rocm/bin/hipcc")
 ARCH = "gfx950"
 CXXFLAGS = [
diff --git a/include/mpt.h b/include/mpt.h
--- a/include/mpt.h
+++ b/include/mpt.h
@@ -433,6 +433,9 @@
 int mpt_comm_gather(MptContext* ctx, int32_t root, int kind, void* dst, int dst_is_device);
 int mpt_set_halo_native(MptContext* ctx, int32_t mode);
 int mpt_set_pipeline(MptContext* ctx, int32_t mode);
+int mpt_set_shade_plans(MptContext* ctx, int32_t mode);
+int mpt_debug_shade_plan(const MptFrame* frame, int32_t bounce, int32_t scene_has_emissives);
+int mpt_debug_shade_plan_ops(int32_t plan);
 typedef struct MptHaloOp {
     int32_t peer;
     int32_t recv;
```
